# LonglongaaaGo/VSPBFR

Measured on AMD Instinct MI355X. Metric: restored 512x512 faces/sec, higher is better.
Workload: dtype f32; 1 GPU; restoration_test.py hot path A+B+C+D, batch 8/GPU, 512x512, 50-step DDPM CodeDiffuser + StyleGAN2 prior + RestoreNet forward, fp32, random-init weights; batch_per_gpu=8, with_style_sample=True, sampler=ddpm, overlap=A+B of batch i+1 on a second HIP stream under C+D of batch i, launch=eager (one host launch per kernel)

## Files before the change

### include/vspbfr_hip.h

```cpp
#ifndef VSPBFR_HIP_H
#define VSPBFR_HIP_H

#include <stdint.h>

#ifdef __cplusplus
extern "C" {
#endif

#define VSP_ABI_VERSION 4

#define VSP_OK 0
#define VSP_EINVAL (-1)
#define VSP_ELAUNCH (-2)
#define VSP_ENOTSUP (-3)

typedef void* vsp_stream_t;

int vsp_abi_version(void);
const char* vsp_last_error(void);
int vsp_device_count(void);
int vsp_struct_size(int which);

int vsp_fused_bias_act_f32(float* out, const float* x, const float* bias, const float* ref, int64_t n,
                           int step_b, int size_b, int act, int grad, float alpha, float scale,
                           vsp_stream_t stream);

typedef struct vsp_fir_epilogue {
  const float* plane_scale;
  const float* noise;
  const float* noise_w;
  const float* act_bias;
  const void* res1;
  const void* res2;
  int channels;
  int act;
  float slope;
  float gain;
  int flags;
} vsp_fir_epilogue;
#define VSP_FIR_SEPARABLE 1

int vsp_upfirdn2d_f32(float* out, const float* x, const float* kernel, int major, int in_h, int in_w,
                      int minor, int kh, int kw, int up_x, int up_y, int down_x, int down_y, int pad_x0,
                      int pad_x1, int pad_y0, int pad_y1, const vsp_fir_epilogue* epi ,
                      vsp_stream_t stream);

typedef struct vsp_conv_params {
  const float* x;
  const float* w;
  float* y;
  int B, Cin, H, W;
  int G, cout_g;
  int OH, OW;
  int KH, KW;
  int stride_y, stride_x;
  int dil[4];
  int pad_y[4];
  int pad_x[4];
  int y_ch, y_coff, y_h, y_w;
  int osy, osx, ooy, oox;
  const float* in_scale;
  int in_scale_bstride;
  const float* in_shift;
  const float* out_scale;
  const float* ch_scale;
  const float* ch_bias;
  int act1;
  const float* bias1;
  float slope1, gain1;
  const float* noise;
  const float* noise_w;
  int act2;
  const float* bias2;
  const float* prelu;
  float slope2, gain2;
  const float* res1;
  const float* res2;
  int res_ch, res_coff;
  int tile_hint;
  int x_ch, x_group_stride;
  int transposed;
  int io_bf16;
  int dil_by_input_quarter;
  int64_t w_bstride;
} vsp_conv_params;

int vsp_conv2d_f32(const vsp_conv_params* p, vsp_stream_t stream);
int vsp_conv2d_winograd_f32(const vsp_conv_params* p, vsp_stream_t stream);
int vsp_conv2d_winograd_chunk(void);
int vsp_conv2d_winograd_mbw(int cout_g);
int vsp_conv2d_winograd4_f32(const vsp_conv_params* p, float* work, size_t work_floats, vsp_stream_t stream);
size_t vsp_winograd4f_weight_floats(int cin, int cout);
int vsp_winograd4f_weight_f32(float* U, const float* wp, int cin, int cout, vsp_stream_t stream);
int vsp_conv2d_winograd4f_f32(const vsp_conv_params* params, vsp_stream_t stream);

size_t vsp_conv2d_winograd4_work_floats(const vsp_conv_params* p);
size_t vsp_winograd4_weight_floats(int cin, int cout);
int vsp_winograd4_weight_f32(float* U, const float* wp, int cin, int cout, vsp_stream_t stream);
int vsp_conv1x1_small_f32(float* y, const float* w, const float* x, const float* bias, int B, int Cout, int Cin, int P, int act,
                          float slope, float gain, vsp_stream_t stream);
int vsp_pack_weight_f32(float* wp, const float* w, int G, int cout_g, int cin, int KH, int KW, int adjoint, int flip, float scale,
                        vsp_stream_t stream);
size_t vsp_winograd_weight_floats(int G, int cin, int cout_g);
int vsp_winograd_weight_f32(float* U, const float* wp, int G, int cin, int cout_g, vsp_stream_t stream);
int vsp_conv2d_num_configs(void);
const char* vsp_conv2d_config_name(int i);

int vsp_conv2d_bf16(const vsp_conv_params* p, vsp_stream_t stream);

int vsp_conv2d_bf16x3(const vsp_conv_params* p, vsp_stream_t stream);

int vsp_conv2d_bf16rv(const vsp_conv_params* p, vsp_stream_t stream);
int vsp_conv2d_bf16dg(const vsp_conv_params* p, vsp_stream_t stream);

typedef struct vsp_gemm_params {
  const float* A;
  const float* Bm;
  float* C;
  int Z, M, N, K;
  int64_t a_zs, a_ms, a_ks;
  int64_t b_zs, b_ns, b_ks;
  int64_t c_zs, c_ms;
  float alpha;
  const float* bias;
  float bias_scale;
  int act;
  float slope, gain;
  int64_t bias_zs;
} vsp_gemm_params;

int vsp_gemm_f32(const vsp_gemm_params* p, vsp_stream_t stream);

int vsp_pixelnorm_dim1_f32(float* out, const float* x, int Z, int R, int C, float eps, vsp_stream_t stream);
int vsp_layernorm_f32(float* out, const float* x, const float* add, const float* gamma, const float* beta,
                      int rows, int cols, float eps, int post, float slope, float gain, vsp_stream_t stream);
int vsp_softmax_lastdim_f32(float* out, const float* x, int rows, int cols, vsp_stream_t stream);
int vsp_softmax_dim1_f32(float* out, const float* x, int Z, int R, int C, vsp_stream_t stream);
int vsp_film_f32(float* out, const float* h, const float* gamma, const float* beta, int64_t n,
                 vsp_stream_t stream);
int vsp_axpby_idx_f32(float* out, const float* x, const float* y, const float* a, const float* b, int idx,
                      int64_t n, vsp_stream_t stream);
int vsp_demod_f32(float* out, const float* style, const float* wsq, int B, int Cin, int Cout, float wscale,
                  float eps, vsp_stream_t stream);
typedef struct {
  const float* w;
  const float* bias;
  const float* wsq;
  float* mod;
  float* demod;
  int64_t src_off;
  int cin, cout;
  float alpha, bias_scale, wscale2;
  int pad_;
} vsp_style_layer;
int vsp_style_plan_f32(const vsp_style_layer* table, int L, const float* src, int B, int64_t bstride, int K, int max_cin, int max_cout,
                       float eps, vsp_stream_t stream);
int vsp_demod_weight_f32(float* out, float* wsq, const float* style, const float* w, int B, int Cin, int Cout, int K, float wscale,
                         float eps, vsp_stream_t stream);
int vsp_demod_weight_bwd_f32(float* dstyle, float* dw, const float* g, const float* out, const float* style, const float* wsq,
                             const float* w, int B, int Cin, int Cout, int K, float wscale, vsp_stream_t stream);
int vsp_demod_weight_bwd_acc_f32(float* dstyle, float* dw, const float* g, int g_stride, const float* out, const float* style,
                                 const float* wsq, const float* w, int B, int Cin, int Cout, int K, float wscale, int accumulate,
                                 vsp_stream_t stream);
int vsp_avgpool2x2_f32(float* out, const float* x, int64_t planes, int OH, int OW, vsp_stream_t stream);
int vsp_upsample_add_f32(float* out, const float* x, const float* y, int64_t planes, int IH, int IW, int OH,
                         int OW, vsp_stream_t stream);
int vsp_plane_mean_f32(float* out, const float* x, int64_t planes, int hw, vsp_stream_t stream);
int vsp_scale_add_f32(float* out, const float* x, const float* gate, const float* y, int64_t planes, int hw,
                      vsp_stream_t stream);
int vsp_subsample_f32(float* out, const float* x, int64_t planes, int IH, int IW, int s, vsp_stream_t stream);
int vsp_quantize_u8_nhwc(uint8_t* out, const float* x, int B, int C, int H, int W, float lo, float hi,
                         vsp_stream_t stream);
#define VSP_WIN_UNIFORM7 7
#define VSP_WIN_GAUSS11 11
size_t vsp_pair_stats_work_bytes(int B, int H, int W, int C, int window);
int vsp_pair_stats_u8(unsigned long long* sse, double* ssim, const uint8_t* a, const uint8_t* b, int B, int H, int W, int C,
                      int window, void* work, vsp_stream_t stream);
int vsp_resize_bilinear_f32(float* out, const float* x, int64_t planes, int IH, int IW, int OH, int OW, vsp_stream_t stream);
int vsp_e4e_codes_f32(float* out, const float* heads, const float* latent_avg, int B, int T, int D, vsp_stream_t stream);
int vsp_rows_concat_f32(float* out, int B, int T, int nseg, const float* const* src, const int* batch_stride, const int* token_stride,
                        const int* width, const int* flip, vsp_stream_t stream);
int vsp_add3_f32(float* out, const float* a, const float* b, const float* c, int64_t n, vsp_stream_t stream);

int vsp_pointwise_f32(float* y, const float* x, const float* w, const float* in_scale, const float* ch_bias,
                      const float* bias1, int act1, const float* bias2, int act2, const float* res, const float* up_src,
                      const float* up_kernel, int W, int B, int Cin, int Cout, int64_t HW, vsp_stream_t stream);

int vsp_tacc_scores_f32(float* score, const float* P, int ldp, int k_off, const float* eQ, const float* wq,
                        int wq_stride, float tfrac, int B, int n_tok, int dim, vsp_stream_t stream);
int vsp_tacc_chan_attn_f32(float* t, const float* P, int ldp, int q2_off, int v2_off, const float* ek,
                           const float* wk, int wk_stride, float tfrac, int B, int n_tok, int dim,
                           vsp_stream_t stream);
int vsp_tacc_tail_f32(float* y, float* pn, const float* P, int ldp, int k_off, int v_off, const float* eQ,
                      const float* wq , float tfrac, const float* t, const float* gamma,
                      const float* beta, const float* xold, const float* c1, const float* c2, int idx, int B, int n_tok,
                      int dim, vsp_stream_t stream);
int vsp_tacc_head_pre_f32(float* out, const float* e, const float* wcol, int w_stride, const float* ln_w,
                          const float* ln_b, int S, int M, int dim, float t_div, vsp_stream_t stream);

typedef struct vsp_tacc_block {
  const float* wcat;
  const float* eQ;
  const float* ek;
  const float* wq;
  const float* wk;
  const float* gamma;
  const float* beta;
  const float* wcat_frag;
} vsp_tacc_block;

typedef struct vsp_tacc_chain_params {
  int B, n_tok, dim, n_blocks;
  const vsp_tacc_block* blocks;
  float* x;
  float* work;
  size_t work_floats;
  int n_steps;
  const int* step;
  const int* coef_idx;
  const float* c1;
  const float* c2;
  float t_div;
  int head_steps;
} vsp_tacc_chain_params;

size_t vsp_tacc_chain_work_floats(int B);
int vsp_tacc_chain_f32(const vsp_tacc_chain_params* p, vsp_stream_t stream);

int vsp_convert_f32_to_bf16(uint16_t* out, const float* x, int64_t n, vsp_stream_t stream);
int vsp_convert_bf16_to_f32(float* out, const uint16_t* x, int64_t n, vsp_stream_t stream);
int vsp_upfirdn2d_bf16(uint16_t* out, const uint16_t* x, const float* kernel, int major, int in_h, int in_w, int minor,
                       int kh, int kw, int up_x, int up_y, int down_x, int down_y, int pad_x0, int pad_x1, int pad_y0,
                       int pad_y1, const vsp_fir_epilogue* epilogue, vsp_stream_t stream);
size_t vsp_modulate_weight_bf16_bytes(int G, int cin, int cout_g);
int vsp_modulate_weight_bf16(uint16_t* out, const float* wp, const float* style, int B, int64_t style_bstride, int G, int cin, int cout_g,
                             vsp_stream_t stream);
int vsp_pointwise_bf16(void* y, const void* x, const float* w, const float* in_scale, const float* ch_bias,
                       const float* bias1, int act1, const float* bias2, int act2, const float* res, const float* up_src,
                       const float* up_kernel, int W, int B, int Cin, int Cout, int64_t HW, vsp_stream_t stream);

typedef struct vsp_conv_wgrad_params {
  const float* x;
  const float* dy;
  float* dw;
  const float* x_scale;
  const float* dy_scale;
  int B, Cin_g, H, W, G, Cout_g, OH, OW, KH, KW, stride, dil, pad;
  int x_ch, x_coff;
  int dy_ch, dy_coff;
  int x_shared;
  int per_group_geometry;
  int dil_g[4], pad_g[4];
  int accumulate;
  float* work;
  size_t work_floats;
  float dw_scale;
} vsp_conv_wgrad_params;
size_t vsp_conv2d_wgrad_work_floats(const vsp_conv_wgrad_params* p);
int vsp_conv2d_wgrad_f32(const vsp_conv_wgrad_params* p, vsp_stream_t stream);
int vsp_plane_dot_f32(float* out, const float* a, const float* b, int64_t planes, int64_t n, vsp_stream_t stream);
int vsp_plane_dot_scale_f32(float* out, float* a, const float* b, const float* scale, int64_t planes, int64_t n, vsp_stream_t stream);
int vsp_noise_bias_act_f32(float* y, const float* x, const float* noise, const float* noise_w, const float* bias, int B, int C,
                           int64_t hw, float slope, float gain, vsp_stream_t stream);
int vsp_noise_dot_f32(float* out, const float* gx, const float* noise, int B, int C, int64_t hw, vsp_stream_t stream);
int vsp_smart_tail_bwd_f32(float* g1, float* db1, float* db2, float* dnw, const float* g, const float* y, const float* noise,
                           const float* noise_w, const float* bias2, int B, int C, int64_t hw, float slope, float gain,
                           vsp_stream_t stream);
int vsp_channel_sum_f32(float* out, const float* x, int B, int C, int64_t hw, vsp_stream_t stream);

int vsp_affine_sample_f32(float* out, const float* x, const float* theta, int B, int C, int IH, int IW, int OH, int OW,
                          vsp_stream_t stream);
int vsp_affine_sample_bwd_f32(float* gx, const float* gout, const float* theta, int B, int C, int IH, int IW, int OH, int OW,
                              vsp_stream_t stream);
int vsp_color_affine_f32(float* y, const float* x, const float* M, const float* t, int B, int64_t HW, vsp_stream_t stream);

int vsp_maxpool2d_f32(float* out, const float* x, int64_t planes, int H, int W, int OH, int OW, int k, int s, int p,
                      vsp_stream_t stream);
int vsp_maxpool2d_bwd_f32(float* dx, const float* dy, const float* x, int64_t planes, int H, int W, int OH, int OW, int k, int s,
                          int p, vsp_stream_t stream);
int vsp_lpips_layer_f32(float* out, const float* f0, const float* f1, const float* w, int B, int C, int HW, vsp_stream_t stream);
int vsp_lpips_layer_bwd_f32(float* df1, const float* f0, const float* f1, const float* w, const float* gout, int B, int C, int HW,
                            vsp_stream_t stream);
int vsp_resize_bilinear_bwd_f32(float* dx, const float* dy, int64_t planes, int IH, int IW, int OH, int OW, vsp_stream_t stream);

#define VSP_NOISE_MAX_SEGMENTS 64
int vsp_keyed_fill_f32(float* out, int B, const int64_t* seg_elems, const int32_t* seg_ids, int n_seg, uint64_t seed,
                       int64_t image_index0, const int64_t* image_index0_dev, int dist, vsp_stream_t stream);

#define VSP_DEGRADE_MAX_KSIZE 41
#define VSP_DEGRADE_MAX_SIZE 2048
#define VSP_DEGRADE_MAX_ITEMS 1024
#define VSP_DEGRADE_HAZE 1
#define VSP_DEGRADE_GREY 2
#define VSP_DEGRADE_NOISE_KEY 0x44475244u

typedef struct vsp_degrade_item {
  int64_t tap_off;
  int64_t pix_off;
  int64_t jpg_off;
  int64_t sample;
  int32_t src;
  int32_t ksize;
  int32_t dh, dw;
  int32_t quality;
  int32_t flags;
  int32_t mcu0;
  int32_t slot;
  float alpha;
  float sigma;
} vsp_degrade_item;

int vsp_degrade_gt_f32(float* out, const uint8_t* hwc, const float* in, const int32_t* grey, int B, int H, int W, vsp_stream_t stream);
int vsp_degrade_blur_f32(float* out, const float* gt, const float* taps, const vsp_degrade_item* items, int n, int B, int H, int W,
                         vsp_stream_t stream);
int vsp_degrade_down_u8(uint8_t* lq, float* pre, const float* blurred, const float* noise, const vsp_degrade_item* items, int n, int H,
                        int W, int max_pixels, uint64_t seed, int64_t step, vsp_stream_t stream);
int vsp_degrade_jpeg_u8(uint8_t* lq, uint8_t* work, const vsp_degrade_item* items, int n, int total_mcus, int max_pixels,
                        vsp_stream_t stream);
int vsp_degrade_up_f32(float* out, const uint8_t* lq, const vsp_degrade_item* items, int n, int H, int W, vsp_stream_t stream);

#define VSP_RESAMPLE_PRECISION_BITS 22
#define VSP_RESAMPLE_MAX_TAPS 97
#define VSP_RESAMPLE_MAX_SIDE 8192
#define VSP_RESAMPLE_MAX_ITEMS 65535
#define VSP_RESAMPLE_FLIP 1
#define VSP_RESAMPLE_COPY 2

typedef struct vsp_resample_item {
  int64_t src_off;
  int64_t work_off;
  int64_t hco, vco;
  int32_t sw, sh;
  int32_t nw, nh;
  int32_t x0, y0;
  int32_t row0, row1;
  int32_t hk, vk;
  int32_t flags;
  int32_t pad_;
} vsp_resample_item;

size_t vsp_lanczos_work_bytes(int rows, int W);
int vsp_lanczos_resize_u8(uint8_t* out_u8, float* out_f32, const uint8_t* src, size_t src_bytes, const int32_t* coef, size_t coef_ints,
                          uint8_t* work, size_t work_bytes, const vsp_resample_item* items, const vsp_resample_item* items_dev, int n,
                          int H, int W, vsp_stream_t stream);

typedef struct vsp_resample_dst {
  int64_t out_off;
  int32_t W, H;
} vsp_resample_dst;

int vsp_lanczos_resize_ragged_u8(uint8_t* out, size_t out_bytes, const uint8_t* src, size_t src_bytes, const int32_t* coef, size_t coef_ints,
                                 uint8_t* work, size_t work_bytes, const vsp_resample_item* items, const vsp_resample_item* items_dev,
                                 const vsp_resample_dst* dst, const vsp_resample_dst* dst_dev, int n, vsp_stream_t stream);

#define VSP_PNG_SEG_ROWS 8
#define VSP_PNG_MAX_ROW_BYTES 3072
#define VSP_PNG_MAX_H 32768
#define VSP_PNG_MAX_BATCH 65535
size_t vsp_png_segment_bound(int rows, int W, int C);
size_t vsp_png_bound(int H, int W, int C);
int vsp_png_encode_u8(uint8_t* out, size_t out_capacity, int32_t* seg_bytes, uint32_t* seg_adler, const uint8_t* src, int B, int H, int W,
                      int C, vsp_stream_t stream);

#define VSP_PNG_RAGGED_SEG_BYTES 24576
#define VSP_PNG_RAGGED_SLOT_BYTES 24588
#define VSP_PNG_RAGGED_MAX_ROW_BYTES (1 << 20)
#define VSP_PNG_RAGGED_MAX_IMAGES 4096
#define VSP_PNG_RAGGED_MAX_SEGMENTS 65535

typedef struct vsp_png_item {
  int64_t src_off;
  int64_t out_off;
  int32_t h, w;
  int32_t seg0;
  int32_t row0;
} vsp_png_item;

int vsp_png_ragged_segments(int H, int W, int C);
size_t vsp_png_ragged_image_bound(int H, int W, int C);
size_t vsp_png_ragged_work_bytes(int64_t segments, int64_t rows);
int vsp_png_encode_ragged_u8(uint8_t* out, size_t out_bytes, int32_t* idat_bytes, uint32_t* seg_adler, uint8_t* work, size_t work_bytes,
                             const uint8_t* src, size_t src_bytes, const vsp_png_item* items, const vsp_png_item* items_dev, int n, int C,
                             vsp_stream_t stream);

#define VSP_NIQE_BLOCK 96
#define VSP_NIQE_FEATURES 36
#define VSP_NIQE_GAMMAS 9801
size_t vsp_niqe_work_bytes(int B, int H, int W, int crop_border);
int vsp_niqe_features_u8(double* features, double* moments_or_null, float* sharpness, const uint8_t* img, int B, int H, int W,
                         int crop_border, const double* rgam_table, void* work, vsp_stream_t stream);

#define VSP_FACE_TILE 32
#define VSP_FACE_MAX_SIDE 8192
#define VSP_FACE_MAX_ITEMS 65535
#define VSP_FACE_MAX_RAMP 65536

typedef struct vsp_face_item {
  int64_t src_off;
  int64_t tab_off;
  int32_t h, w;
  int32_t x0, y0;
  int32_t nx, ny;
} vsp_face_item;

typedef struct vsp_face_tile {
  int64_t dst_off;
  int32_t h, w;
  int32_t x0, y0;
  int32_t face0;
  int32_t nfaces;
} vsp_face_tile;

int vsp_face_crop_u8(uint8_t* out_u8, float* out_f32, const uint8_t* src, size_t src_bytes, const int32_t* tables, const int32_t* tables_dev,
                     size_t table_ints, const vsp_face_item* items, const vsp_face_item* items_dev, int n, int S, int border_r, int border_g,
                     int border_b, vsp_stream_t stream);
int vsp_face_paste_u8(uint8_t* photos, size_t photo_bytes, const uint8_t* crops, size_t crop_bytes, const int32_t* tables,
                      const int32_t* tables_dev, size_t table_ints, const vsp_face_item* items, const vsp_face_item* items_dev, int n, int S,
                      const vsp_face_tile* tiles, const vsp_face_tile* tiles_dev, int ntiles, const int32_t* tile_faces,
                      const int32_t* tile_faces_dev, size_t tile_face_ints, const uint16_t* ramp, const uint16_t* ramp_dev, int ramp_len,
                      vsp_stream_t stream);

#define VSP_FACE_AA_MAX_REACH 23
#define VSP_FACE_AA_MAX_RANGE (1 << 18)

typedef struct vsp_face_aa_item {
  int64_t src_off;
  int64_t tab_off;
  int64_t fwd_off;
  int32_t h, w;
  int32_t x0, y0;
  int32_t nx, ny;
  int32_t sx0, sy0;
  int32_t snx, sny;
  int32_t reach;
  int32_t pad_;
} vsp_face_aa_item;

int vsp_face_crop_aa_u8(uint8_t* out_u8, float* out_f32, const uint8_t* src, size_t src_bytes, const int32_t* tables, const int32_t* tables_dev,
                        size_t table_ints, const int32_t* fwd, const int32_t* fwd_dev, size_t fwd_ints, const vsp_face_aa_item* items,
                        const vsp_face_aa_item* items_dev, int n, int S, int border_r, int border_g, int border_b, vsp_stream_t stream);
int vsp_face_paste_aa_u8(uint8_t* photos, size_t photo_bytes, const uint8_t* crops, size_t crop_bytes, const int32_t* tables,
                         const int32_t* tables_dev, size_t table_ints, const int32_t* fwd, const int32_t* fwd_dev, size_t fwd_ints,
                         const vsp_face_aa_item* items, const vsp_face_aa_item* items_dev, int n, int S, const vsp_face_tile* tiles,
                         const vsp_face_tile* tiles_dev, int ntiles, const int32_t* tile_faces, const int32_t* tile_faces_dev,
                         size_t tile_face_ints, const uint16_t* ramp, const uint16_t* ramp_dev, int ramp_len, vsp_stream_t stream);

#define VSP_COLOR_FIX_STATS 0
#define VSP_COLOR_FIX_WAVELET 1
#define VSP_COLOR_FIX_MAX_LEVELS 6
#define VSP_COLOR_FIX_STATS_MAX_SIDE 1024

int vsp_color_fix_u8(const uint8_t* crop, const uint8_t* restored, uint8_t* out, int F, int S, int mode, int levels,
                     const vsp_face_item* items, const vsp_face_item* items_dev, const int32_t* tables, const int32_t* tables_dev,
                     size_t table_ints, void* scratch, size_t scratch_bytes, vsp_stream_t stream);

#define VSP_JPEG_444 0
#define VSP_JPEG_420 2
#define VSP_JPEG_MAX_ITEMS 65535
#define VSP_JPEG_BLOCK_BOUND 416

typedef struct vsp_jpeg_item {
  int64_t src_off;
  int64_t out_off;
  int32_t h, w;
  int32_t interval0;
  int32_t pad_;
} vsp_jpeg_item;

int vsp_jpeg_intervals(int h, int w, int restart, int subsampling);
size_t vsp_jpeg_interval_bound(int mcus, int subsampling);
size_t vsp_jpeg_image_bound(int h, int w, int restart, int subsampling);
int vsp_jpeg_encode_u8(uint8_t* out, size_t out_bytes, int32_t* totals, uint8_t* work, size_t work_bytes, int32_t* interval_ws,
                       const uint8_t* src, size_t src_bytes, const vsp_jpeg_item* items, const vsp_jpeg_item* items_dev, int n,
                       int quality, int subsampling, int restart, vsp_stream_t stream);

#define VSP_JPEG_DEC_TABLE_BYTES 1824
#define VSP_JPEG_DEC_MAX_SCAN_BYTES 0x0FFFFFFF
#define VSP_JPEG_DEC_COEF_LIMIT 16383
#define VSP_JPEG_DEC_NO_EOI 1
#define VSP_JPEG_DEC_STRAY_MARKER 2
#define VSP_JPEG_DEC_RST_ORDER 4
#define VSP_JPEG_DEC_RST_COUNT 8
#define VSP_JPEG_DEC_BAD_CODE 16
#define VSP_JPEG_DEC_BAD_CATEGORY 32
#define VSP_JPEG_DEC_RUN 64
#define VSP_JPEG_DEC_BLOCK_COUNT 128
#define VSP_JPEG_DEC_COEF_RANGE 256

typedef struct vsp_jpeg_dec_item {
  int64_t in_off;
  int64_t out_off;
  int64_t work_off;
  int32_t in_len;
  int32_t h, w;
  int32_t subsampling;
  int32_t restart;
  int32_t interval0;
} vsp_jpeg_dec_item;

size_t vsp_jpeg_decode_work_bytes(int h, int w, int in_len, int subsampling, int restart, int sub_bytes);
int vsp_jpeg_decode_u8(uint8_t* out, size_t out_bytes, int32_t* status, int32_t* rounds, uint8_t* work, size_t work_bytes, const uint8_t* in,
                       size_t in_bytes, const vsp_jpeg_dec_item* items, const vsp_jpeg_dec_item* items_dev, const uint8_t* tables,
                       const uint8_t* tables_dev, int n, int sub_bytes, vsp_stream_t stream);

#ifdef __cplusplus
}
#endif
#endif
```

### vspbfr_amd/_lib.py

```python
import ctypes as C
import os

import torch

from .photo import FaceAAItem, FaceItem, FaceTile
from .resample import ResampleDst, ResampleItem

_HERE = os.path.dirname(os.path.abspath(__file__))
LIB_PATH = os.environ.get("VSPBFR_HIP_LIB", os.path.join(_HERE, "lib", "libvspbfr_hip.so"))



def tune_env(name, default=None):
    if os.environ.get("VSP_TUNE", "0") in ("", "0"):
        return default
    return os.environ.get(name, default)


ABI_VERSION = 4
c_float_p = C.c_void_p


class FirEpilogue(C.Structure):
    _fields_ = [
        ("plane_scale", C.c_void_p), ("noise", C.c_void_p), ("noise_w", C.c_void_p), ("act_bias", C.c_void_p),
        ("res1", C.c_void_p), ("res2", C.c_void_p),
        ("channels", C.c_int), ("act", C.c_int), ("slope", C.c_float), ("gain", C.c_float), ("flags", C.c_int),
    ]


FIR_SEPARABLE = 1


class ConvParams(C.Structure):
    _fields_ = [
        ("x", C.c_void_p), ("w", C.c_void_p), ("y", C.c_void_p),
        ("B", C.c_int), ("Cin", C.c_int), ("H", C.c_int), ("W", C.c_int),
        ("G", C.c_int), ("cout_g", C.c_int),
        ("OH", C.c_int), ("OW", C.c_int),
        ("KH", C.c_int), ("KW", C.c_int),
        ("stride_y", C.c_int), ("stride_x", C.c_int),
        ("dil", C.c_int * 4), ("pad_y", C.c_int * 4), ("pad_x", C.c_int * 4),
        ("y_ch", C.c_int), ("y_coff", C.c_int), ("y_h", C.c_int), ("y_w", C.c_int),
        ("osy", C.c_int), ("osx", C.c_int), ("ooy", C.c_int), ("oox", C.c_int),
        ("in_scale", C.c_void_p), ("in_scale_bstride", C.c_int), ("in_shift", C.c_void_p),
        ("out_scale", C.c_void_p), ("ch_scale", C.c_void_p), ("ch_bias", C.c_void_p),
        ("act1", C.c_int), ("bias1", C.c_void_p), ("slope1", C.c_float), ("gain1", C.c_float),
        ("noise", C.c_void_p), ("noise_w", C.c_void_p),
        ("act2", C.c_int), ("bias2", C.c_void_p), ("prelu", C.c_void_p), ("slope2", C.c_float), ("gain2", C.c_float),
        ("res1", C.c_void_p), ("res2", C.c_void_p), ("res_ch", C.c_int), ("res_coff", C.c_int),
        ("tile_hint", C.c_int), ("x_ch", C.c_int), ("x_group_stride", C.c_int), ("transposed", C.c_int),
        ("io_bf16", C.c_int),
        ("dil_by_input_quarter", C.c_int),
        ("w_bstride", C.c_int64),
    ]


class ConvWgradParams(C.Structure):
    _fields_ = [("x", C.c_void_p), ("dy", C.c_void_p), ("dw", C.c_void_p), ("x_scale", C.c_void_p), ("dy_scale", C.c_void_p)] + [
        (n, C.c_int) for n in ("B", "Cin_g", "H", "W", "G", "Cout_g", "OH", "OW", "KH", "KW", "stride", "dil", "pad", "x_ch", "x_coff", "dy_ch",
                               "dy_coff", "x_shared", "per_group_geometry")] + [("dil_g", C.c_int * 4), ("pad_g", C.c_int * 4),
                                                                                ("accumulate", C.c_int), ("work", C.c_void_p),
                                                                                ("work_floats", C.c_size_t), ("dw_scale", C.c_float)]


class TaccBlock(C.Structure):
    _fields_ = [(n, C.c_void_p) for n in ("wcat", "eQ", "ek", "wq", "wk", "gamma", "beta", "wcat_frag")]


class TaccChainParams(C.Structure):
    _fields_ = [
        ("B", C.c_int), ("n_tok", C.c_int), ("dim", C.c_int), ("n_blocks", C.c_int),
        ("blocks", C.POINTER(TaccBlock)), ("x", C.c_void_p), ("work", C.c_void_p), ("work_floats", C.c_size_t),
        ("n_steps", C.c_int), ("step", C.POINTER(C.c_int)), ("coef_idx", C.POINTER(C.c_int)),
        ("c1", C.c_void_p), ("c2", C.c_void_p), ("t_div", C.c_float), ("head_steps", C.c_int),
    ]


class GemmParams(C.Structure):
    _fields_ = [
        ("A", C.c_void_p), ("Bm", C.c_void_p), ("C", C.c_void_p),
        ("Z", C.c_int), ("M", C.c_int), ("N", C.c_int), ("K", C.c_int),
        ("a_zs", C.c_int64), ("a_ms", C.c_int64), ("a_ks", C.c_int64),
        ("b_zs", C.c_int64), ("b_ns", C.c_int64), ("b_ks", C.c_int64),
        ("c_zs", C.c_int64), ("c_ms", C.c_int64),
        ("alpha", C.c_float), ("bias", C.c_void_p), ("bias_scale", C.c_float),
        ("act", C.c_int), ("slope", C.c_float), ("gain", C.c_float), ("bias_zs", C.c_int64),
    ]


class DegradeItem(C.Structure):
    _fields_ = [("tap_off", C.c_int64), ("pix_off", C.c_int64), ("jpg_off", C.c_int64), ("sample", C.c_int64)] + [
        (n, C.c_int32) for n in ("src", "ksize", "dh", "dw", "quality", "flags", "mcu0", "slot")] + [("alpha", C.c_float), ("sigma", C.c_float)]


class JpegItem(C.Structure):
    _fields_ = [("src_off", C.c_int64), ("out_off", C.c_int64), ("h", C.c_int32), ("w", C.c_int32), ("interval0", C.c_int32), ("pad_", C.c_int32)]


class PngItem(C.Structure):
    _fields_ = [("src_off", C.c_int64), ("out_off", C.c_int64), ("h", C.c_int32), ("w", C.c_int32), ("seg0", C.c_int32), ("row0", C.c_int32)]


class JpegDecItem(C.Structure):
    _fields_ = [("in_off", C.c_int64), ("out_off", C.c_int64), ("work_off", C.c_int64)] + [
        (n, C.c_int32) for n in ("in_len", "h", "w", "subsampling", "restart", "interval0")]


DEGRADE_HAZE, DEGRADE_GREY = 1, 2
DEGRADE_MAX_KSIZE, DEGRADE_MAX_SIZE, DEGRADE_MAX_ITEMS = 41, 2048, 1024
WIN_UNIFORM7, WIN_GAUSS11 = 7, 11

_i, _i64, _f, _p = C.c_int, C.c_int64, C.c_float, C.c_void_p

SIGNATURES = {
    "vsp_abi_version": [],
    "vsp_device_count": [],
    "vsp_struct_size": [_i],
    "vsp_fused_bias_act_f32": [_p, _p, _p, _p, _i64, _i, _i, _i, _i, _f, _f, _p],
    "vsp_upfirdn2d_f32": [_p, _p, _p] + [_i] * 14 + [C.POINTER(FirEpilogue), _p],
    "vsp_conv2d_f32": [C.POINTER(ConvParams), _p],
    "vsp_conv2d_num_configs": [],
    "vsp_gemm_f32": [C.POINTER(GemmParams), _p],
    "vsp_pixelnorm_dim1_f32": [_p, _p, _i, _i, _i, _f, _p],
    "vsp_layernorm_f32": [_p, _p, _p, _p, _p, _i, _i, _f, _i, _f, _f, _p],
    "vsp_softmax_lastdim_f32": [_p, _p, _i, _i, _p],
    "vsp_softmax_dim1_f32": [_p, _p, _i, _i, _i, _p],
    "vsp_film_f32": [_p, _p, _p, _p, _i64, _p],
    "vsp_axpby_idx_f32": [_p, _p, _p, _p, _p, _i, _i64, _p],
    "vsp_demod_f32": [_p, _p, _p, _i, _i, _i, _f, _f, _p],
    "vsp_style_plan_f32": [_p, _i, _p, _i, _i64, _i, _i, _i, _f, _p],
    "vsp_demod_weight_f32": [_p, _p, _p, _p, _i, _i, _i, _i, _f, _f, _p],
    "vsp_demod_weight_bwd_f32": [_p, _p, _p, _p, _p, _p, _p, _i, _i, _i, _i, _f, _p],
    "vsp_demod_weight_bwd_acc_f32": [_p, _p, _p, _i, _p, _p, _p, _p, _i, _i, _i, _i, _f, _i, _p],
    "vsp_avgpool2x2_f32": [_p, _p, _i64, _i, _i, _p],
    "vsp_upsample_add_f32": [_p, _p, _p, _i64, _i, _i, _i, _i, _p],
    "vsp_e4e_codes_f32": [_p, _p, _p, _i, _i, _i, _p],
    "vsp_rows_concat_f32": [_p, _i, _i, _i, C.POINTER(C.c_void_p), C.POINTER(_i), C.POINTER(_i), C.POINTER(_i), C.POINTER(_i), _p],
    "vsp_resize_bilinear_f32": [_p, _p, _i64, _i, _i, _i, _i, _p],
    "vsp_plane_mean_f32": [_p, _p, _i64, _i, _p],
    "vsp_scale_add_f32": [_p, _p, _p, _p, _i64, _i, _p],
    "vsp_subsample_f32": [_p, _p, _i64, _i, _i, _i, _p],
    "vsp_add3_f32": [_p, _p, _p, _p, _i64, _p],
    "vsp_pointwise_f32": [_p, _p, _p, _p, _p, _p, _i, _p, _i, _p, _p, _p, _i, _i, _i, _i, _i64, _p],
    "vsp_quantize_u8_nhwc": [_p, _p, _i, _i, _i, _i, _f, _f, _p],
    "vsp_tacc_scores_f32": [_p, _p, _i, _i, _p, _p, _i, _f, _i, _i, _i, _p],
    "vsp_tacc_chan_attn_f32": [_p, _p, _i, _i, _i, _p, _p, _i, _f, _i, _i, _i, _p],
    "vsp_tacc_tail_f32": [_p, _p, _p, _i, _i, _i, _p, _p, _f, _p, _p, _p, _p, _p, _p, _i, _i, _i, _i, _p],
    "vsp_tacc_head_pre_f32": [_p, _p, _p, _i, _p, _p, _i, _i, _i, _f, _p],
    "vsp_tacc_chain_f32": [_p, _p],
    "vsp_conv2d_winograd_f32": [_p, _p],
    "vsp_conv2d_bf16": [_p, _p],
    "vsp_conv2d_bf16x3": [_p, _p],
    "vsp_conv2d_bf16rv": [_p, _p],
    "vsp_conv2d_bf16dg": [_p, _p],
    "vsp_affine_sample_f32": [_p, _p, _p, _i, _i, _i, _i, _i, _i, _p],
    "vsp_affine_sample_bwd_f32": [_p, _p, _p, _i, _i, _i, _i, _i, _i, _p],
    "vsp_color_affine_f32": [_p, _p, _p, _p, _i, _i64, _p],
    "vsp_maxpool2d_f32": [_p, _p, _i64, _i, _i, _i, _i, _i, _i, _i, _p],
    "vsp_maxpool2d_bwd_f32": [_p, _p, _p, _i64, _i, _i, _i, _i, _i, _i, _i, _p],
    "vsp_lpips_layer_f32": [_p, _p, _p, _p, _i, _i, _i, _p],
    "vsp_lpips_layer_bwd_f32": [_p, _p, _p, _p, _p, _i, _i, _i, _p],
    "vsp_resize_bilinear_bwd_f32": [_p, _p, _i64, _i, _i, _i, _i, _p],
    "vsp_conv2d_wgrad_f32": [C.POINTER(ConvWgradParams), _p],
    "vsp_plane_dot_f32": [_p, _p, _p, _i64, _i64, _p],
    "vsp_channel_sum_f32": [_p, _p, _i, _i, _i64, _p],
    "vsp_noise_bias_act_f32": [_p, _p, _p, _p, _p, _i, _i, _i64, C.c_float, C.c_float, _p],
    "vsp_noise_dot_f32": [_p, _p, _p, _i, _i, _i64, _p],
    "vsp_smart_tail_bwd_f32": [_p, _p, _p, _p, _p, _p, _p, _p, _p, _i, _i, _i64, C.c_float, C.c_float, _p],
    "vsp_plane_dot_scale_f32": [_p, _p, _p, _p, _i64, _i64, _p],
    "vsp_convert_f32_to_bf16": [_p, _p, _i64, _p],
    "vsp_convert_bf16_to_f32": [_p, _p, _i64, _p],
    "vsp_upfirdn2d_bf16": [_p, _p, _p] + [_i] * 14 + [C.POINTER(FirEpilogue), _p],
    "vsp_pointwise_bf16": [_p, _p, _p, _p, _p, _p, _i, _p, _i, _p, _p, _p, _i, _i, _i, _i, _i64, _p],
    "vsp_keyed_fill_f32": [_p, _i, C.POINTER(C.c_int64), C.POINTER(C.c_int32), _i, C.c_uint64, _i64, _p, _i, _p],
    "vsp_conv1x1_small_f32": [_p, _p, _p, _p, _i, _i, _i, _i, _i, _f, _f, _p],
    "vsp_pack_weight_f32": [_p, _p, _i, _i, _i, _i, _i, _i, _i, _f, _p],
    "vsp_winograd_weight_f32": [_p, _p, _i, _i, _i, _p],
    "vsp_winograd4_weight_f32": [_p, _p, _i, _i, _p],
    "vsp_conv2d_winograd4_f32": [_p, _p, C.c_size_t, _p],
    "vsp_winograd4f_weight_f32": [_p, _p, _i, _i, _p],
    "vsp_conv2d_winograd4f_f32": [_p, _p],
    "vsp_modulate_weight_bf16": [_p, _p, _p, _i, _i64, _i, _i, _i, _p],
    "vsp_conv2d_winograd_chunk": [],
    "vsp_conv2d_winograd_mbw": [_i],
    "vsp_degrade_gt_f32": [_p, _p, _p, _p, _i, _i, _i, _p],
    "vsp_degrade_blur_f32": [_p, _p, _p, _p, _i, _i, _i, _i, _p],
    "vsp_degrade_down_u8": [_p, _p, _p, _p, _p, _i, _i, _i, _i, C.c_uint64, _i64, _p],
    "vsp_degrade_jpeg_u8": [_p, _p, _p, _i, _i, _i, _p],
    "vsp_degrade_up_f32": [_p, _p, _p, _i, _i, _i, _p],
    "vsp_pair_stats_u8": [_p, _p, _p, _p, _i, _i, _i, _i, _i, _p, _p],
    "vsp_lanczos_resize_u8": [_p, _p, _p, C.c_size_t, _p, C.c_size_t, _p, C.c_size_t, _p, _p, _i, _i, _i, _p],
    "vsp_lanczos_resize_ragged_u8": [_p, C.c_size_t, _p, C.c_size_t, _p, C.c_size_t, _p, C.c_size_t, _p, _p, _p, _p, _i, _p],
    "vsp_png_encode_u8": [_p, C.c_size_t, _p, _p, _p, _i, _i, _i, _i, _p],
    "vsp_png_ragged_segments": [_i, _i, _i],
    "vsp_png_encode_ragged_u8": [_p, C.c_size_t, _p, _p, _p, C.c_size_t, _p, C.c_size_t, _p, _p, _i, _i, _p],
    "vsp_niqe_features_u8": [_p, _p, _p, _p, _i, _i, _i, _i, _p, _p, _p],
    "vsp_face_crop_u8": [_p, _p, _p, C.c_size_t, _p, _p, C.c_size_t, _p, _p, _i, _i, _i, _i, _i, _p],
    "vsp_face_paste_u8": [_p, C.c_size_t, _p, C.c_size_t, _p, _p, C.c_size_t, _p, _p, _i, _i, _p, _p, _i, _p, _p, C.c_size_t, _p, _p, _i, _p],
    "vsp_face_crop_aa_u8": [_p, _p, _p, C.c_size_t, _p, _p, C.c_size_t, _p, _p, C.c_size_t, _p, _p, _i, _i, _i, _i, _i, _p],
    "vsp_face_paste_aa_u8": [_p, C.c_size_t, _p, C.c_size_t, _p, _p, C.c_size_t, _p, _p, C.c_size_t, _p, _p, _i, _i, _p, _p, _i, _p, _p,
                             C.c_size_t, _p, _p, _i, _p],
    "vsp_color_fix_u8": [_p, _p, _p, _i, _i, _i, _i, _p, _p, _p, _p, C.c_size_t, _p, C.c_size_t, _p],
    "vsp_jpeg_intervals": [_i, _i, _i, _i],
    "vsp_jpeg_encode_u8": [_p, C.c_size_t, _p, _p, C.c_size_t, _p, _p, C.c_size_t, _p, _p, _i, _i, _i, _i, _p],
    "vsp_jpeg_decode_u8": [_p, C.c_size_t, _p, _p, _p, C.c_size_t, _p, C.c_size_t, _p, _p, _p, _p, _i, _i, _p],
}
_CHARP = {"vsp_last_error": [], "vsp_conv2d_config_name": [_i]}
_SIZET = {"vsp_tacc_chain_work_floats": [_i], "vsp_conv2d_wgrad_work_floats": [C.POINTER(ConvWgradParams)],
          "vsp_winograd_weight_floats": [_i, _i, _i], "vsp_winograd4_weight_floats": [_i, _i], "vsp_winograd4f_weight_floats": [_i, _i],
          "vsp_conv2d_winograd4_work_floats": [_p], "vsp_modulate_weight_bf16_bytes": [_i, _i, _i],
          "vsp_pair_stats_work_bytes": [_i, _i, _i, _i, _i], "vsp_lanczos_work_bytes": [_i, _i],
          "vsp_png_segment_bound": [_i, _i, _i], "vsp_png_bound": [_i, _i, _i],
          "vsp_png_ragged_image_bound": [_i, _i, _i], "vsp_png_ragged_work_bytes": [_i64, _i64],
          "vsp_niqe_work_bytes": [_i, _i, _i, _i],
          "vsp_jpeg_interval_bound": [_i, _i], "vsp_jpeg_image_bound": [_i, _i, _i, _i],
          "vsp_jpeg_decode_work_bytes": [_i, _i, _i, _i, _i, _i]}


def _load():
    if not os.path.exists(LIB_PATH):
        raise ImportError(
            f"vspbfr_amd: HIP library not found at {LIB_PATH}. Build it with `python -c 'import __graft_entry__ as g; "
            f"g.build()'` or `make -C vspbfr_amd/csrc`; there is no CPU fallback.")
    lib = C.CDLL(LIB_PATH)
    for name, args in SIGNATURES.items():
        fn = getattr(lib, name)
        fn.argtypes = args
        fn.restype = C.c_int
    for name, args in _CHARP.items():
        fn = getattr(lib, name)
        fn.argtypes = args
        fn.restype = C.c_char_p
    for name, args in _SIZET.items():
        fn = getattr(lib, name)
        fn.argtypes = args
        fn.restype = C.c_size_t
    if lib.vsp_abi_version() != ABI_VERSION:
        raise ImportError(f"vspbfr_amd: ABI version {lib.vsp_abi_version()} != {ABI_VERSION}")
    for which, st in ((0, FirEpilogue), (1, ConvParams), (2, GemmParams), (3, TaccBlock), (4, TaccChainParams),
                      (5, ConvWgradParams), (6, DegradeItem), (7, ResampleItem), (8, FaceItem), (9, FaceTile), (10, FaceAAItem), (11, JpegItem), (12, JpegDecItem),
                      (13, ResampleDst), (14, PngItem)):
        if lib.vsp_struct_size(which) != C.sizeof(st):
            raise ImportError(f"vspbfr_amd: struct layout mismatch for {st.__name__}: "
                              f"C {lib.vsp_struct_size(which)} vs ctypes {C.sizeof(st)}")
    return lib


lib = _load()


def last_error():
    return lib.vsp_last_error().decode("utf-8", "replace")


def check(rc, what):
    if rc != 0:
        raise RuntimeError(f"{what} failed (code {rc}): {last_error()}")


def exported_symbols():
    return sorted(list(SIGNATURES) + list(_CHARP) + list(_SIZET))
```

### vspbfr_amd/csrc/conv_igemm.hip

```cpp
#include "conv_kernel.h"
#include <cstdlib>
#include <cstring>

namespace vspconv {
extern const Cfg kCfgsA[];
extern const int kNumA;
extern const Cfg kCfgsB[];
extern const int kNumB;
extern const Cfg kCfgsC[];
extern const int kNumC;
extern const Cfg kCfgsD[];
extern const int kNumD;
extern const Cfg kCfgsE[];
extern const int kNumE;
extern const Cfg kCfgsF[];
extern const int kNumF;
extern const Cfg kCfgsG[];
extern const int kNumG;
extern const Cfg kCfgsP[];
extern const int kNumP;
}

namespace {

using vspconv::Cfg;
using vspconv::ConvK;

__device__ float kConst[8] = {1.f, 0.f, 1.f, 0.f, 0.f, 0.f, 0.f, 0.f};

constexpr int kMaxCfgs = 192;
static Cfg kCfgs[kMaxCfgs];
static int kNumCfgs = 0;

static void build_table() {
  if (kNumCfgs) return;
  using namespace vspconv;
  const struct { const Cfg* cfgs; int count; } units[] = {{kCfgsA, kNumA}, {kCfgsB, kNumB}, {kCfgsC, kNumC}, {kCfgsD, kNumD},
                                                          {kCfgsE, kNumE}, {kCfgsF, kNumF}, {kCfgsG, kNumG}, {kCfgsP, kNumP}};
  int n = 0;
  for (const auto& u : units)
    for (int i = 0; i < u.count && n < kMaxCfgs; ++i) kCfgs[n++] = u.cfgs[i];
  kNumCfgs = n;
}

constexpr size_t kMaxLds = 100 * 1024;
constexpr size_t kMaxLdsPipe = 160 * 1024;

struct Plan {
  int cfg;
  int tw_log2, th, tiles_x, tiles_y, co_tiles;
  bool dg;
  int strip_col, strip_row;
  size_t lds;
  int ps;
};

static int ilog2_ceil(int v) {
  int l = 0;
  while ((1 << l) < v) ++l;
  return l;
}

static int host_round_pitch(int n, int odd) {
  if (odd) return n | 1;
  int p = (n & ~31) + 16;
  return p >= n ? p : p + 32;
}

struct CfgKind {
  bool tc, dg, kg, fg;
};
static CfgKind cfg_kind(const Cfg& k) {
  const size_t n = strlen(k.name);
  const char last = k.name[n - 1];
  return {last == 't', last == 'd', last == 'a', n >= 2 && k.name[n - 2] == 'f'};
}

static bool make_plan(const vsp_conv_params& p, int c, Plan* out) {
  const Cfg& k = kCfgs[c];
  const CfgKind kind = cfg_kind(k);
  const bool tc = kind.tc;
  if (tc != (p.transposed != 0)) return false;
  const bool kg = kind.kg;
  if (kg != (p.dil_by_input_quarter != 0)) return false;
  const bool dg = kind.dg || kg;
  if (dg) {
    if (p.G != 4 || p.x_group_stride != 0 || p.stride_y != 1 || p.stride_x != 1 || p.KH != 3 || p.KW != 3) return false;
    for (int g = 0; g < 4; ++g)
      if (p.pad_y[g] != p.dil[g] || p.pad_x[g] != p.dil[g]) return false;
  }
  const int CO_T = 16 * k.MB * k.WM, NPIX = tc ? 16 * k.WN * (k.NB / 4) : 16 * k.NB * k.WN;
  const int WS = (CO_T % 32 == 0) ? CO_T + 16 : CO_T;
  int twl = ilog2_ceil(p.OW);
  int cap = NPIX >= 256 ? 5 : 4;
  if (k.PF == 3 && dg) cap = NPIX >= 512 ? 5 : 4;
  if (twl > cap) twl = cap;
  if ((1 << twl) > NPIX) twl = ilog2_ceil(NPIX);
  const bool fg = k.PF == 3 && kind.fg;
  if (fg) {
    twl = 4;
    if (!dg || p.dil[0] != 1 || p.dil[1] != 2 || p.dil[2] != 4 || p.dil[3] != 8) return false;
  }
  const int TW = 1 << twl, TH = NPIX / TW;
  int dmax = 1;
  for (int g = 0; g < (p.G > 4 ? 1 : p.G); ++g) dmax = p.dil[g] > dmax ? p.dil[g] : dmax;
  const int PH = tc ? TH + 1 : (TH - 1) * p.stride_y + (p.KH - 1) * dmax + 1;
  const int PW = tc ? TW + 1 : (TW - 1) * p.stride_x + (p.KW - 1) * dmax + 1;
  if (PW > 256 || PH * PW >= 65536) return false;
  int plane = PH * PW;
  out->strip_col = -1;
  out->strip_row = 0;
  out->tiles_x = (p.OW + TW - 1) / TW;
  out->tiles_y = (p.OH + TH - 1) / TH;
  if (tc && (NPIX <= 128 || k.PF == 3) && p.H % TH == 0 && p.W % TW == 0) {
    out->tiles_x = p.W / TW;
    out->tiles_y = p.H / TH;
    out->strip_col = (p.H + NPIX - 1) / NPIX;
    out->strip_row = (p.W + 1 + NPIX - 1) / NPIX;
    if ((NPIX + 1) * 2 > plane) plane = (NPIX + 1) * 2;
  }
  if (k.PF == 3) {
    if (p.KH != 3 || p.KW != 3 || p.cout_g % 4 != 0 || !vsp::aligned16(p.w) || p.in_shift || p.Cin % k.CK != 0) return false;
    if (kg && (p.Cin % 16 != 0 || (p.Cin / 4) % k.CK != 0)) return false;
    const int NW = k.WM * k.WN, wpc = k.CK >= NW ? 1 : NW / k.CK;
    const int nrow = (plane + 63) / 64;
    const int ps = host_round_pitch(k.PMAX * wpc * 64, !tc && p.stride_x != 1);
    if (nrow > k.PMAX * wpc) return false;
    const size_t lds = 2 * ((size_t)9 * k.CK * WS + (size_t)k.CK * ps) * sizeof(float);
    if (lds > kMaxLdsPipe) return false;
    out->cfg = c; out->tw_log2 = twl; out->th = TH;
    out->co_tiles = dg ? (p.cout_g + 15) / 16 : (p.cout_g + CO_T - 1) / CO_T;
    out->dg = dg; out->lds = lds; out->ps = ps;
    return true;
  }
  const int PS = host_round_pitch(plane, !tc && p.stride_x != 1);
  if (k.PF == 2 && (p.in_shift || p.cout_g % 4 != 0 || !vsp::aligned16(p.w) || p.KH * p.KW > 9)) return false;
  size_t lds = ((size_t)p.KH * p.KW * k.CK * WS + (size_t)(k.PF == 2 ? 2 : 1) * k.CK * PS) * sizeof(float);
  const size_t red = (size_t)(k.WK - 1) * k.WM * k.WN * k.MB * k.NB * 4 * 64 * sizeof(float);
  if (red > lds) lds = red;
  if (lds > kMaxLds) return false;
  out->cfg = c;
  out->tw_log2 = twl;
  out->th = TH;
  out->co_tiles = dg ? (p.cout_g + 15) / 16 : (p.cout_g + CO_T - 1) / CO_T;
  out->dg = dg;
  out->lds = lds;
  return true;
}

static double plan_cost(const vsp_conv_params& p, const Plan& pl) {
  const Cfg& k = kCfgs[pl.cfg];
  const int waves = k.WM * k.WN * k.WK;
  const double blocks = ((double)pl.tiles_x * pl.tiles_y + (pl.strip_col > 0 ? pl.strip_col + pl.strip_row : 0)) * pl.co_tiles * (pl.dg ? 1 : p.G) * p.B;
  const int cin_pad = (p.Cin + k.CK - 1) / k.CK * k.CK;
  const double ksteps = (double)p.KH * p.KW * cin_pad / 4.0;
  const double mfma_cyc = ksteps * k.MB * k.NB * 32.0 / k.WK;
  const double reads = ksteps * (k.MB + k.NB) * 8.0 / k.WK;
  const double chunks = (double)cin_pad / k.CK;
  const double stage = chunks * 2500.0;
  int per_cu = (int)(160 * 1024 / (pl.lds + 1024));
  if (per_cu > 4) per_cu = 4;
  if (per_cu < 1) per_cu = 1;
  const double wps = per_cu * waves / 4.0;
  double t_block = mfma_cyc * (wps < 1.0 ? 1.0 : wps) + (wps >= 2.0 ? 0.15 : 1.0) * stage + 0.05 * reads;
  const double slots = 256.0 * per_cu;
  const double rounds = blocks / slots;
  const double full = (rounds < 1.0) ? 1.0 : rounds;
  if (rounds < 1.0) {
    const double occ = blocks / 256.0;
    const double w = occ * waves / 4.0;
    t_block = mfma_cyc * (w < 1.0 ? 1.0 : w) + stage + 0.05 * reads;
  }
  return full * t_block;
}

static const float* device_consts() {
  static const float* cache[64] = {};
  int dev = 0;
  if (hipGetDevice(&dev) != hipSuccess || dev < 0 || dev >= 64) {
    vsp::set_error("hipGetDevice failed");
    return nullptr;
  }
  if (!cache[dev]) {
    void* ptr = nullptr;
    hipError_t e = hipGetSymbolAddress(&ptr, HIP_SYMBOL(kConst));
    if (e != hipSuccess) {
      vsp::set_error("hipGetSymbolAddress(kConst): %s", hipGetErrorString(e));
      return nullptr;
    }
    const float init[8] = {1.f, 0.f, 1.f, 0.f, 0.2f, 0.01f, 0.f, 0.f};
    e = hipMemcpy(ptr, init, sizeof(init), hipMemcpyHostToDevice);
    if (e != hipSuccess) {
      vsp::set_error("hipMemcpy(kConst): %s", hipGetErrorString(e));
      return nullptr;
    }
    cache[dev] = static_cast<const float*>(ptr);
  }
  return cache[dev];
}

static const float* slope_slot(const float* kc, float slope) {
  if (slope == 0.2f) return kc + 4;
  if (slope == 0.01f) return kc + 5;
  if (slope == 1.f) return kc;
  if (slope == 0.f) return kc + 1;
  return nullptr;
}

}

static int validate_conv(const vsp_conv_params& p, int* x_ch_out, bool* empty, bool allow_w_bstride = false) {
  *empty = false;
  VSP_REQUIRE(p.x && p.w && p.y, "conv2d: null tensor pointer");
  VSP_REQUIRE(p.B >= 0 && p.Cin >= 1 && p.H >= 1 && p.W >= 1, "conv2d: bad input dims B=%d Cin=%d H=%d W=%d", p.B,
              p.Cin, p.H, p.W);
  VSP_REQUIRE(p.G >= 1 && p.G <= 1024 && p.cout_g >= 1, "conv2d: bad group spec G=%d cout_g=%d", p.G, p.cout_g);
  VSP_REQUIRE(p.x_group_stride >= 0 && p.x_ch >= 0, "conv2d: negative x_ch / x_group_stride");
  VSP_REQUIRE(p.w_bstride == 0 || allow_w_bstride, "conv2d: per-image weights (w_bstride) are served by vsp_conv2d_bf16 with io_bf16 = 1 only");
  const int x_ch = p.x_ch > 0 ? p.x_ch : p.Cin;
  VSP_REQUIRE((int64_t)(p.G - 1) * p.x_group_stride + p.Cin <= x_ch, "conv2d: group input channels exceed x_ch=%d", x_ch);
  VSP_REQUIRE(p.x_group_stride == 0 || !p.in_shift, "conv2d: an input shift is not supported with grouped input");
  VSP_REQUIRE(p.KH >= 1 && p.KW >= 1 && p.KH * p.KW <= 49, "conv2d: unsupported kernel %dx%d", p.KH, p.KW);
  VSP_REQUIRE(p.stride_y >= 1 && p.stride_x >= 1 && p.stride_x <= 2 && p.stride_y <= 2, "conv2d: stride must be 1 or 2");
  VSP_REQUIRE(p.dil_by_input_quarter == 0 || (p.dil_by_input_quarter == 1 && p.G == 4 && p.x_group_stride == 0 && p.Cin % 16 == 0 && !p.transposed),
              "conv2d: dil_by_input_quarter needs G = 4 blocks of output channels over one shared input with Cin %% 16 == 0");
  VSP_REQUIRE(p.OH >= 0 && p.OW >= 0, "conv2d: negative output size");
  VSP_REQUIRE(p.osy >= 1 && p.osx >= 1 && p.ooy >= 0 && p.oox >= 0, "conv2d: bad output stride/offset");
  VSP_REQUIRE(!p.noise || p.noise_w, "conv2d: noise given without noise_w");
  VSP_REQUIRE(p.act2 != 2 || p.prelu, "conv2d: act2=prelu without slopes");
  for (int g = 0; g < (p.G > 4 ? 1 : p.G); ++g) VSP_REQUIRE(p.dil[g] >= 1, "conv2d: dilation must be >= 1");
  if (p.B == 0 || p.OH == 0 || p.OW == 0) {
    *empty = true;
    return VSP_OK;
  }
  const int Cout = p.G * p.cout_g;
  VSP_REQUIRE(p.y_coff >= 0 && p.y_coff + Cout <= p.y_ch, "conv2d: output channel window [%d,%d) outside %d", p.y_coff,
              p.y_coff + Cout, p.y_ch);
  VSP_REQUIRE((p.OH - 1) * p.osy + p.ooy < p.y_h && (p.OW - 1) * p.osx + p.oox < p.y_w,
              "conv2d: output positions exceed the %dx%d output tensor", p.y_h, p.y_w);
  VSP_REQUIRE((int64_t)p.y_ch * p.y_h * p.y_w < ((int64_t)1 << 31) && (int64_t)x_ch * p.H * p.W < ((int64_t)1 << 31),
              "conv2d: one image must hold fewer than 2^31 elements");
  if (p.res1 || p.res2)
    VSP_REQUIRE(p.res_coff >= 0 && p.res_coff + Cout <= p.res_ch, "conv2d: residual channel window out of range");

  *x_ch_out = x_ch;
  return VSP_OK;
}

static int fill_convk(const vsp_conv_params& p, int x_ch, ConvK& q) {
  q.x = p.x; q.w = p.w; q.y = p.y;
  q.B = p.B; q.Cin = p.Cin; q.H = p.H; q.W = p.W; q.G = p.G; q.cout_g = p.cout_g;
  q.OH = p.OH; q.OW = p.OW; q.KH = p.KH; q.KW = p.KW; q.sy = p.stride_y; q.sx = p.stride_x;
  for (int g = 0; g < 4; ++g) { q.dil[g] = p.dil[g]; q.pady[g] = p.pad_y[g]; q.padx[g] = p.pad_x[g]; }
  q.y_ch = p.y_ch; q.y_coff = p.y_coff; q.y_h = p.y_h; q.y_w = p.y_w;
  q.osy = p.osy; q.osx = p.osx; q.ooy = p.ooy; q.oox = p.oox;
  q.in_scale = p.in_scale; q.in_scale_bstride = p.in_scale_bstride; q.in_shift = p.in_shift;
  const float* kc = device_consts();
  VSP_REQUIRE(kc != nullptr, "conv2d: cannot resolve device constants: %s", vsp_last_error());
  const float* kOne = kc;
  const float* kZero = kc + 1;
  auto sel = [](const float* ptr, const float* dflt, const float** outp, int* outs) {
    *outp = ptr ? ptr : dflt;
    *outs = ptr ? 1 : 0;
  };
  sel(p.out_scale, kOne, &q.osp, &q.oss);
  sel(p.ch_scale, kOne, &q.csp, &q.css);
  sel(p.ch_bias, kZero, &q.cbp, &q.cbs);
  sel(p.act1 ? p.bias1 : nullptr, kZero, &q.b1p, &q.b1s);
  q.s1 = p.act1 ? p.slope1 : 1.f;
  q.g1 = p.act1 ? p.gain1 : 1.f;
  sel(p.noise, kZero, &q.nzp, &q.nzs);
  q.nwp = p.noise ? p.noise_w : kZero;
  sel(p.act2 == 1 ? p.bias2 : nullptr, kZero, &q.b2p, &q.b2s);
  if (p.act2 == 2) {
    q.s2p = p.prelu; q.s2s = 1; q.g2 = 1.f;
  } else if (p.act2 == 1) {
    const float* slot = slope_slot(kc, p.slope2);
    VSP_REQUIRE(slot != nullptr, "conv2d: unsupported act2 slope %g (supported: 0.2, 0.01, 0, 1)", p.slope2);
    q.s2p = slot; q.s2s = 0; q.g2 = p.gain2;
  } else {
    q.s2p = kOne; q.s2s = 0; q.g2 = 1.f;
  }
  sel(p.res1, kZero, &q.r1p, &q.r1s);
  sel(p.res2, kZero, &q.r2p, &q.r2s);
  q.res_ch = p.res_ch; q.res_coff = p.res_coff;
  q.x_ch = x_ch;
  q.x_gs = p.x_group_stride;
  return VSP_OK;
}

static int conv_front(const vsp_conv_params& p, ConvK& q, bool* empty, bool allow_w_bstride = false) {
  int x_ch = 0;
  if (int rc = validate_conv(p, &x_ch, empty, allow_w_bstride)) return rc;
  if (*empty) return VSP_OK;
  if (int rc = fill_convk(p, x_ch, q)) return rc;
  static const int dbg = vsp::tune_env("VSP_CONV_DBG") ? atoi(vsp::tune_env("VSP_CONV_DBG")) : 0;
  q.dbg = dbg;
  const float* kc = device_consts();
  const bool affine = p.in_shift != nullptr, style = p.in_scale && !affine, scaled = p.in_scale && affine;
  q.wtp = style ? p.in_scale : kc;       q.wt_cs = style ? 1 : 0;    q.wt_bs = style ? p.in_scale_bstride : 0;
  q.wcp = scaled ? p.in_scale : kc;      q.wc_cs = scaled ? 1 : 0;   q.wc_bs = scaled ? p.in_scale_bstride : 0;
  q.wshp = affine ? p.in_shift : kc + 1; q.wsh_cs = affine ? 1 : 0;
  q.bf_isc_s = p.in_scale ? 1 : 0;
  q.bf_ish_s = affine ? 1 : 0;
  return VSP_OK;
}

static int require_dilation_groups(const char* who, const vsp_conv_params& p, int n, int dmax, bool pow2) {
  for (int g = 0; g < n; ++g)
    VSP_REQUIRE(p.dil[g] >= 1 && p.dil[g] <= dmax && (!pow2 || (p.dil[g] & (p.dil[g] - 1)) == 0) && p.pad_y[g] == p.dil[g] && p.pad_x[g] == p.dil[g],
                "%s: group %d needs a dilation of %s and padding = dilation (got dilation %d, padding %d/%d)", who, g,
                pow2 ? "1, 2, 4 or 8" : "1 to 64", p.dil[g], p.pad_y[g], p.pad_x[g]);
  return VSP_OK;
}

static int require_dense_output(const char* who, const vsp_conv_params& p, bool same_size) {
  const bool dense = p.osy == 1 && p.osx == 1 && p.ooy == 0 && p.oox == 0;
  if (!same_size) {
    VSP_REQUIRE(dense, "%s: dense output only", who);
    return VSP_OK;
  }
  VSP_REQUIRE(dense && p.OH == p.H && p.OW == p.W, "%s: dense same-size output only: the output size must equal the input size", who);
  return VSP_OK;
}

static int require_input_under_2gib(const char* who, const vsp_conv_params& p) {
  VSP_REQUIRE((double)(p.x_ch > 0 ? p.x_ch : p.Cin) * p.H * p.W * 4 < 2147483648.0,
              "%s: one input image must be smaller than 2 GiB (32-bit buffer offsets)", who);
  return VSP_OK;
}

static int normalise_transposed(const char* who, vsp_conv_params& p, bool exact) {
  VSP_REQUIRE(p.KH == 3 && p.KW == 3 && p.G == 1, "%s: transposed mode needs a 3x3 kernel and G = 1", who);
  VSP_REQUIRE(!p.noise && !p.res1 && !p.res2, "%s: transposed mode has no noise / residual epilogue", who);
  const int oh = 2 * p.H + 1, ow = 2 * p.W + 1;
  VSP_REQUIRE(exact ? (p.y_h == oh && p.y_w == ow) : (p.y_h >= oh && p.y_w >= ow), "%s: transposed output must %s (2H+1)x(2W+1)", who,
              exact ? "be" : "hold");
  p.stride_y = p.stride_x = 1;
  p.dil[0] = 1;
  p.pad_y[0] = p.pad_x[0] = 1;
  p.OH = p.H + 1;
  p.OW = p.W + 1;
  p.osy = p.osx = 2;
  p.ooy = p.oox = 0;
  return VSP_OK;
}

extern "C" int vsp_conv2d_num_configs(void) {
  build_table();
  return kNumCfgs + 1;
}
extern "C" const char* vsp_conv2d_config_name(int i) {
  build_table();
  return (i >= 0 && i < kNumCfgs) ? kCfgs[i].name : (i == kNumCfgs ? "smallmap" : "");
}

extern "C" int vsp_conv2d_winograd_chunk(void) { return vspconv::wino_chunk(); }
extern "C" int vsp_conv2d_winograd_mbw(int cout_g) { return vspconv::wino_mbw(cout_g); }

extern "C" int vsp_conv2d_winograd_f32(const vsp_conv_params* pp, vsp_stream_t stream) {
  const char* who = "conv2d_winograd";
  VSP_REQUIRE(pp != nullptr, "conv2d_winograd: null params");
  const vsp_conv_params& p = *pp;
  VSP_REQUIRE(!p.transposed && p.G >= 1 && p.G <= 4 && p.KH == 3 && p.KW == 3 && p.stride_y == 1 && p.stride_x == 1 &&
                  p.x_group_stride == 0,
              "conv2d_winograd: only 3x3, stride 1, at most four groups over one shared input");
  if (int rc = require_dilation_groups(who, p, p.G, 8, true)) return rc;
  VSP_REQUIRE(p.io_bf16 == 0, "conv2d_winograd: fp32 activations only (io_bf16 is served by vsp_conv2d_bf16)");
  VSP_REQUIRE(p.dil_by_input_quarter == 0, "conv2d_winograd: dil_by_input_quarter is served by vsp_conv2d_f32");
  if (int rc = require_dense_output(who, p, true)) return rc;
  VSP_REQUIRE(vsp::aligned16(p.w), "conv2d_winograd: transformed weights must be 16-byte aligned");
  VSP_REQUIRE((int64_t)16 * p.Cin * p.cout_g < ((int64_t)1 << 31), "conv2d_winograd: weight tensor too large");
  if (int rc = require_input_under_2gib(who, p)) return rc;
  VSP_REQUIRE(p.tile_hint >= 0 && p.tile_hint <= 3, "conv2d_winograd: tile_hint names the kernel form: 0 automatic, 1 task list, 2 row owner, 3 register-resident U");
  ConvK q{};
  bool empty = false;
  if (int rc = conv_front(p, q, &empty)) return rc;
  if (empty) return VSP_OK;
  if (int rc = vspconv::wino_launch(q, p.tile_hint, vsp::as_stream(stream))) return rc;
  return vsp::check_launch(who);
}

extern "C" size_t vsp_winograd4_weight_floats(int cin, int cout) { return vspconv::wino4_weight_floats(cin, cout); }

extern "C" int vsp_winograd4_weight_f32(float* U, const float* wp, int cin, int cout, vsp_stream_t stream) {
  VSP_REQUIRE(U && wp && cin >= 1 && cout >= 1, "winograd4_weight: bad arguments");
  if (int rc = vspconv::wino4_weight_launch(U, wp, cin, cout, vsp::as_stream(stream))) return rc;
  return vsp::check_launch("winograd4_weight");
}

extern "C" size_t vsp_conv2d_winograd4_work_floats(const vsp_conv_params* pp) {
  return pp ? vspconv::wino4_work_floats(pp->B, pp->Cin, pp->H, pp->W) : 0;
}

extern "C" int vsp_conv2d_winograd4_f32(const vsp_conv_params* pp, float* work, size_t work_floats, vsp_stream_t stream) {
  const char* who = "conv2d_winograd4";
  VSP_REQUIRE(pp != nullptr && work != nullptr, "conv2d_winograd4: null params / work buffer");
  const vsp_conv_params& p = *pp;
  VSP_REQUIRE(!p.transposed && p.G == 1 && p.KH == 3 && p.KW == 3 && p.stride_y == 1 && p.stride_x == 1 && p.dil[0] == 1 &&
                  p.pad_y[0] == 1 && p.pad_x[0] == 1,
              "conv2d_winograd4: one group, 3x3, stride 1, dilation 1, padding 1");
  VSP_REQUIRE(p.io_bf16 == 0 && p.dil_by_input_quarter == 0 && p.in_shift == nullptr, "conv2d_winograd4: fp32, no affine input shift");
  if (int rc = require_dense_output(who, p, true)) return rc;
  VSP_REQUIRE(vsp::aligned16(p.w) && vsp::aligned16(work), "conv2d_winograd4: weights and work buffer must be 16-byte aligned");
  VSP_REQUIRE(work_floats >= vspconv::wino4_work_floats(p.B, p.Cin, p.H, p.W), "conv2d_winograd4: work buffer too small");
  VSP_REQUIRE((int64_t)vspconv::wino4_work_floats(1, p.Cin, p.H, p.W) * 4 < ((int64_t)1 << 40), "conv2d_winograd4: image too large");
  ConvK q{};
  bool empty = false;
  if (int rc = conv_front(p, q, &empty)) return rc;
  if (empty) return VSP_OK;
  if (!vspconv::wino4_eligible(q))
    return vsp::fail(VSP_ENOTSUP, "conv2d_winograd4: needs Cin %% 4 == 0, H, W %% 4 == 0, dense 16-byte aligned output / noise / residual planes");
  if (int rc = vspconv::wino4_launch(q, work, p.in_scale, p.in_scale ? p.in_scale_bstride : 0, vsp::as_stream(stream))) return rc;
  return vsp::check_launch(who);
}

extern "C" size_t vsp_winograd4f_weight_floats(int cin, int cout) { return vspconv::wino4f_weight_floats(cin, cout); }

extern "C" int vsp_winograd4f_weight_f32(float* U, const float* wp, int cin, int cout, vsp_stream_t stream) {
  VSP_REQUIRE(U && wp && cin >= 1 && cout >= 1, "winograd4f_weight: bad arguments");
  if (int rc = vspconv::wino4f_weight_launch(U, wp, cin, cout, vsp::as_stream(stream))) return rc;
  return vsp::check_launch("winograd4f_weight");
}

extern "C" int vsp_conv2d_winograd4f_f32(const vsp_conv_params* pp, vsp_stream_t stream) {
  const char* who = "conv2d_winograd4f";
  VSP_REQUIRE(pp != nullptr, "conv2d_winograd4f: null params");
  const vsp_conv_params& p = *pp;
  VSP_REQUIRE(!p.transposed && p.G >= 1 && p.G <= 4 && p.KH == 3 && p.KW == 3 && p.stride_y == 1 && p.stride_x == 1,
              "conv2d_winograd4f: 3x3, stride 1, one group or up to four dilation groups over one shared input");
  if (int rc = require_dilation_groups(who, p, p.G, 8, true)) return rc;
  VSP_REQUIRE(p.io_bf16 == 0 && p.dil_by_input_quarter == 0 && p.in_shift == nullptr, "conv2d_winograd4f: fp32, no affine input shift");
  if (int rc = require_dense_output(who, p, true)) return rc;
  VSP_REQUIRE(vsp::aligned16(p.w), "conv2d_winograd4f: weights must be 16-byte aligned");
  ConvK q{};
  bool empty = false;
  if (int rc = conv_front(p, q, &empty)) return rc;
  if (empty) return VSP_OK;
  if (!vspconv::wino4f_eligible(q))
    return vsp::fail(VSP_ENOTSUP, "conv2d_winograd4f: needs Cin %% 8 == 0 (<= 512), H, W %% (4 x dilation) == 0, W >= 16, groups over one shared input, dense 16-byte aligned input / output / noise / residual planes < 2 GiB per image");
  if (int rc = vspconv::wino4f_launch(q, vsp::as_stream(stream))) return rc;
  return vsp::check_launch(who);
}

enum Bf16Kernel { kBf16General, kBf16Split, kBf16RowVector, kBf16DilationGroups };
static int conv2d_bf16_impl(const vsp_conv_params* pp, vsp_stream_t stream, Bf16Kernel kern);
extern "C" int vsp_conv2d_bf16(const vsp_conv_params* pp, vsp_stream_t stream) { return conv2d_bf16_impl(pp, stream, kBf16General); }
extern "C" int vsp_conv2d_bf16x3(const vsp_conv_params* pp, vsp_stream_t stream) { return conv2d_bf16_impl(pp, stream, kBf16Split); }
extern "C" int vsp_conv2d_bf16rv(const vsp_conv_params* pp, vsp_stream_t stream) { return conv2d_bf16_impl(pp, stream, kBf16RowVector); }
extern "C" int vsp_conv2d_bf16dg(const vsp_conv_params* pp, vsp_stream_t stream) { return conv2d_bf16_impl(pp, stream, kBf16DilationGroups); }

static int conv2d_bf16_impl(const vsp_conv_params* pp, vsp_stream_t stream, Bf16Kernel kern) {
  const char* who = "conv2d_bf16";
  VSP_REQUIRE(pp != nullptr, "conv2d_bf16: null params");
  vsp_conv_params pcopy = *pp;
  int mode = 0;
  VSP_REQUIRE(pcopy.KH == 3 && pcopy.KW == 3 && pcopy.G >= 1, "conv2d_bf16: 3x3 kernels only");
  if (pcopy.transposed) {
    mode = 2;
    if (int rc = normalise_transposed(who, pcopy, true)) return rc;
  } else if (pcopy.stride_y == 2 && pcopy.stride_x == 2) {
    mode = 1;
    VSP_REQUIRE(pcopy.dil[0] == 1 && pcopy.pad_y[0] == pcopy.pad_x[0] && (pcopy.pad_y[0] == 0 || pcopy.pad_y[0] == 1),
                "conv2d_bf16: stride 2 needs dilation 1 and padding 0 or 1");
    VSP_REQUIRE(pcopy.G == 1 || pcopy.x_group_stride > 0, "conv2d_bf16: stride-2 groups need their own input slices");
    VSP_REQUIRE(pcopy.OH <= (pcopy.H + 2 * pcopy.pad_y[0] - 3) / 2 + 1 && pcopy.OW <= (pcopy.W + 2 * pcopy.pad_x[0] - 3) / 2 + 1,
                "conv2d_bf16: output larger than the stride-2 convolution of the input");
  } else {
    VSP_REQUIRE(pcopy.stride_y == 1 && pcopy.stride_x == 1, "conv2d_bf16: stride must be 1 or 2");
    VSP_REQUIRE(pcopy.G <= 4 || pcopy.x_group_stride > 0, "conv2d_bf16: more than four groups need their own input slices");
    if (int rc = require_dilation_groups(who, pcopy, pcopy.G > 4 ? 1 : pcopy.G, 64, false)) return rc;
  }
  const vsp_conv_params& p = pcopy;
  if (mode != 2)
    if (int rc = require_dense_output(who, p, mode == 0)) return rc;
  VSP_REQUIRE(vsp::aligned16(p.w), "conv2d_bf16: packed weights must be 16-byte aligned");
  VSP_REQUIRE(p.Cin % 8 == 0, "conv2d_bf16: Cin must be a multiple of 8 (got %d)", p.Cin);
  if (int rc = require_input_under_2gib(who, p)) return rc;
  if (p.w_bstride != 0) {
    VSP_REQUIRE(kern == kBf16General && p.io_bf16 == 1, "conv2d_bf16: per-image weights need the general bf16 kernel with bf16 activations");
    VSP_REQUIRE(p.w_bstride > 0 && p.w_bstride % 16 == 0, "conv2d_bf16: w_bstride must be a positive multiple of 16 bytes");
    VSP_REQUIRE(!p.in_scale && !p.in_shift, "conv2d_bf16: per-image weights carry the style: in_scale / in_shift must be NULL");
    VSP_REQUIRE((p.W & 1) == 0 && (reinterpret_cast<uintptr_t>(p.x) & 3) == 0, "conv2d_bf16: per-image weights need even rows (pixel-pair staging)");
  }
  VSP_REQUIRE((int64_t)p.G * p.cout_g <= 65535 && p.B <= 65535, "conv2d_bf16: grid too large");
  VSP_REQUIRE(!(kern == kBf16Split && p.io_bf16), "conv2d_bf16x3: the split-precision form keeps fp32 activations (io_bf16 = 0)");
  VSP_REQUIRE(p.io_bf16 == 0 || p.io_bf16 == 1, "conv2d_bf16: io_bf16 must be 0 or 1");
  VSP_REQUIRE(p.dil_by_input_quarter == 0, "conv2d_bf16: dil_by_input_quarter is served by vsp_conv2d_f32");
  ConvK q{};
  bool empty = false;
  if (int rc = conv_front(p, q, &empty, true)) return rc;
  if (empty) return VSP_OK;
  q.in_scale = p.in_shift ? q.wcp : q.wtp;
  q.in_scale_bstride = p.in_shift ? q.wc_bs : q.wt_bs;
  q.in_shift = q.wshp;
  q.io_bf16 = p.io_bf16;
  q.w_bs = p.w_bstride / 16;
  const hipStream_t s = vsp::as_stream(stream);
  switch (kern) {
    case kBf16DilationGroups:
      if (mode != 0 || !vspconv::bf16dg_eligible(q)) return VSP_ENOTSUP;
      if (int rc = vspconv::bf16dg_launch(q, p.act1 != 0 || p.act2 != 0 || p.noise != nullptr, s)) return rc;
      return vsp::check_launch("conv2d_bf16dg");
    case kBf16RowVector:
      if (mode != 0 || !vspconv::bf16rv_eligible(q)) return VSP_ENOTSUP;
      if (int rc = vspconv::bf16rv_launch(q, p.tile_hint, s)) return rc;
      return vsp::check_launch("conv2d_bf16rv");
    case kBf16Split:
      if (int rc = vspconv::bf16_launch_split(q, mode, p.tile_hint, s)) return rc;
      return vsp::check_launch("conv2d_bf16x3");
    case kBf16General: break;
  }
  if (int rc = vspconv::bf16_launch(q, mode, p.tile_hint, s)) return rc;
  return vsp::check_launch(who);
}

extern "C" int vsp_conv2d_f32(const vsp_conv_params* pp, vsp_stream_t stream) {
  const char* who = "conv2d";
  VSP_REQUIRE(pp != nullptr, "conv2d: null params");
  VSP_REQUIRE(pp->io_bf16 == 0, "conv2d: fp32 activations only (io_bf16 is served by vsp_conv2d_bf16)");
  build_table();
  vsp_conv_params pcopy = *pp;
  if (pcopy.transposed)
    if (int rc = normalise_transposed(who, pcopy, false)) return rc;
  const vsp_conv_params& p = pcopy;
  if (int rc = require_input_under_2gib(who, p)) return rc;
  VSP_REQUIRE((double)p.KH * p.KW * p.Cin * p.cout_g * 4 < 2147483648.0, "conv2d: one group's weights must be smaller than 2 GiB (32-bit buffer offsets)");
  ConvK q{};
  bool empty = false;
  if (int rc = conv_front(p, q, &empty)) return rc;
  if (empty) return VSP_OK;
  {
    const int sm = kNumCfgs + 1;
    const bool named = p.tile_hint == sm, preferred = p.tile_hint == -sm;
    const bool guess = p.tile_hint == 0 && (int64_t)p.B * p.OH * p.OW <= 256 && (int64_t)p.Cin * p.KH * p.KW >= 1024;
    if ((named || preferred || guess) && !p.dil_by_input_quarter) {
      if (vspconv::smallmap_eligible(q, p.transposed != 0)) return vspconv::smallmap_launch(q, vsp::as_stream(stream));
      VSP_REQUIRE(!named, "conv2d: configuration smallmap does not fit this problem (Cin %% 16 == 0, at most 8192 output positions, not transposed)");
    }
  }
  Plan best{};
  bool found = false;
  if (p.tile_hint > 0) {
    VSP_REQUIRE(p.tile_hint <= kNumCfgs, "conv2d: tile_hint %d out of range", p.tile_hint);
    found = make_plan(p, p.tile_hint - 1, &best);
    VSP_REQUIRE(found, "conv2d: configuration %s does not fit this problem", kCfgs[p.tile_hint - 1].name);
  } else if (p.tile_hint < 0 && -p.tile_hint <= kNumCfgs) {
    found = make_plan(p, -p.tile_hint - 1, &best);
  }
  if (!found) {
    double best_cost = 0.0;
    for (int c = 0; c < kNumCfgs; ++c) {
      Plan pl{};
      const CfgKind kind = cfg_kind(kCfgs[c]);
      if (p.dil_by_input_quarter ? !kind.kg : (kind.dg || kCfgs[c].PF == 3)) continue;
      if (!make_plan(p, c, &pl)) continue;
      const double cost = p.dil_by_input_quarter ? (double)c : plan_cost(p, pl);
      if (!found || cost < best_cost) {
        best = pl;
        best_cost = cost;
        found = true;
      }
    }
    if (!found) return vsp::fail(VSP_ENOTSUP, "conv2d: no tile configuration fits (KH=%d dil=%d)", p.KH, p.dil[0]);
  }
  const Cfg& k = kCfgs[best.cfg];
  const int CO_T = 16 * k.MB * k.WM;
  const int64_t gy = best.dg ? best.co_tiles : (int64_t)best.co_tiles * p.G;
  VSP_REQUIRE(gy <= 65535 && p.B <= 65535, "conv2d: grid too large");

  q.tw_log2 = best.tw_log2; q.th = best.th; q.tiles_x = best.tiles_x; q.tiles_y = best.tiles_y;
  q.strip_col = best.strip_col;
  q.co_tiles = best.co_tiles;
  q.w_vec4 = (p.cout_g % 4 == 0) && (CO_T % 4 == 0) && vsp::aligned16(p.w) ? 1 : 0;
  q.ps_odd = !p.transposed && p.stride_x != 1;

  if (k.PF == 3) {
    q.bf_plane = best.ps;
    q.wcp = q.wtp;  q.wc_cs = q.wt_cs;  q.wc_bs = q.wt_bs;
  }
  if (best.lds > 64 * 1024) {
    static vsp::LdsAttrOnce raised[kMaxCfgs];
    if (int rc = raised[best.cfg].ensure(reinterpret_cast<const void*>(k.kern), (int)(k.PF == 3 ? kMaxLdsPipe : kMaxLds), "conv2d")) return rc;
  }
  q.wg_order = (q.dbg & 0x1000000) ? 0 : 1;
  if (k.PF == 3 && p.G == 1 && q.wg_order == 1 && !(q.dbg & 0x20000)) {
    const int64_t wtile = (int64_t)p.Cin * p.KH * p.KW * CO_T * 4, wall = wtile * best.co_tiles;
    const int64_t xall = (int64_t)p.B * p.Cin * p.H * p.W * 4;
    if (wall > 16 * 1024 * 1024 && best.co_tiles >= 4 && wall * 2 > xall / 8) {
      int cgs = (int)((int64_t)(2 * 1024 * 1024) / wtile);
      q.wg_cgs = cgs < 1 ? 1 : (cgs > best.co_tiles ? best.co_tiles : cgs);
      q.wg_order = 2;
    }
  }
  dim3 grid((unsigned)(best.tiles_x * best.tiles_y + (best.strip_col > 0 ? best.strip_col + best.strip_row : 0)), (unsigned)gy,
            (unsigned)p.B);
  dim3 block(64 * k.WM * k.WN * k.WK);
  hipLaunchKernelGGL(k.kern, grid, block, best.lds, vsp::as_stream(stream), q);
  return vsp::check_launch("conv2d");
}
```

### vspbfr_amd/csrc/conv_kernel.h

```cpp
#pragma once
#include "vsp_common.h"

namespace vspconv {

using f32x4 = __attribute__((ext_vector_type(4))) float;

struct ConvK {
  const float* x;
  const float* w;
  float* y;
  int B, Cin, H, W, G, cout_g, OH, OW, KH, KW, sy, sx;
  int dil[4], pady[4], padx[4];
  int y_ch, y_coff, y_h, y_w, osy, osx, ooy, oox;
  const float* in_scale;
  int in_scale_bstride;
  const float* in_shift;
  const float* osp; int oss;
  const float* csp; int css;
  const float* cbp; int cbs;
  const float* b1p; int b1s;
  float s1, g1;
  const float* nzp; int nzs;
  const float* nwp;
  const float* b2p; int b2s;
  const float* s2p; int s2s;
  float g2;
  const float* r1p; int r1s;
  const float* r2p; int r2s;
  int res_ch, res_coff;
  int tw_log2, th, tiles_x, tiles_y, co_tiles;
  int w_vec4;
  int ps_odd;
  int x_ch, x_gs;
  int strip_col;
  int dbg;
  int bf_pitch, bf_plane;
  int bf_isc_s, bf_ish_s;
  int wg_order;
  const float* wtp; int wt_cs, wt_bs;
  const float* wcp; int wc_cs, wc_bs;
  const float* wshp; int wsh_cs;
  int io_bf16;
  int64_t w_bs;
  int bf_tab;
  int wg_cgs;
  int rv_copad, rv_cbase, rv_ctot;
};

__device__ __forceinline__ int round_pitch(int n, int odd) {
  if (odd) return n | 1;
  int p = (n & ~31) + 16;
  return p >= n ? p : p + 32;
}

template <int MB, int NB, int WM, int WN, int CK, int WK, int PMAX, int PF, int OCC, bool TC = false, bool DG = false>
__global__ __launch_bounds__(64 * WM * WN * WK, OCC) void conv_igemm_kernel(const ConvK p) {
  static_assert(!TC || (NB % 4 == 0 && WK == 1), "transposed mode: N-blocks come in groups of four sub-pixel phases");
  constexpr int NP = TC ? NB / 4 : NB;
  static_assert(!DG || (MB == 4 && WM == 1 && WK == 1 && !TC), "dilation-group mode: M-block = group");
  constexpr int NT = 64 * WM * WN * WK;
  constexpr int CO_T = 16 * MB * WM;
  constexpr int WS = (CO_T % 32 == 0) ? CO_T + 16 : CO_T;
  extern __shared__ __attribute__((aligned(16))) float smem[];

  const int tid = threadIdx.x;
  const int lane = tid & 63;
  const int wave = __builtin_amdgcn_readfirstlane(tid >> 6);
  const int wk = wave / (WM * WN);
  const int wmn = wave - wk * (WM * WN);
  const int wm = wmn / WN, wn = wmn % WN;
  const int lr = lane & 15;
  const int kq = lane >> 4;

  int tile = blockIdx.x, by = blockIdx.y, bz = blockIdx.z;
  if (p.wg_order == 1) {
    const int GX = gridDim.x, GY = gridDim.y, GN = GX * GY, GT = GN * gridDim.z;
    const int wgid = blockIdx.x + GX * (blockIdx.y + GY * blockIdx.z);
    const int xcd = wgid & 7, xq = GT >> 3, xr = GT & 7;
    const int lid = (xcd < xr ? xcd * (xq + 1) : xr * (xq + 1) + (xcd - xr) * xq) + (wgid >> 3);
    bz = lid / GN;
    const int lrem = lid - bz * GN;
    tile = lrem / GY;
    by = lrem - tile * GY;
  }
  const int tx_i = tile % p.tiles_x, ty_i = tile / p.tiles_x;
  const int g = DG ? 0 : by / p.co_tiles;
  const int co0 = DG ? by * 16 : (by % p.co_tiles) * CO_T;
  const int b = bz;

  int twl = p.tw_log2, TH = p.th, oy0 = ty_i * p.th, ox0 = tx_i << p.tw_log2;
  int mlim = p.H + 1;
  if (TC && p.strip_col >= 0) {
    constexpr int NPIXB = 16 * WN * (NB / 4);
    mlim = p.H;
    int j = tile - p.tiles_x * p.tiles_y;
    if (j >= p.strip_col) {
      j -= p.strip_col;
      twl = __builtin_ctz(NPIXB); TH = 1; oy0 = p.H; ox0 = j * NPIXB; mlim = p.H + 1;
    } else if (j >= 0) {
      twl = 0; TH = NPIXB; oy0 = j * NPIXB; ox0 = p.W;
    }
  }
  const int TW = 1 << twl;
  const int gi = p.G > 4 ? 0 : g;
  const int D = DG ? max(max(p.dil[0], p.dil[1]), max(p.dil[2], p.dil[3])) : p.dil[gi];
  const int T = p.KH * p.KW;
  const int PH = TC ? TH + 1 : (TH - 1) * p.sy + (p.KH - 1) * D + 1;
  const int PW = TC ? TW + 1 : (TW - 1) * p.sx + (p.KW - 1) * D + 1;
  const int PS = round_pitch(PH * PW, p.ps_odd);
  const int iy0 = TC ? oy0 - 1 : DG ? oy0 - D : oy0 * p.sy - p.pady[gi];
  const int ix0 = TC ? ox0 - 1 : DG ? ox0 - D : ox0 * p.sx - p.padx[gi];

  float* Wl = smem;
  float* Pl = smem + T * CK * WS;

  int pixoff[NP];
#pragma unroll
  for (int nb = 0; nb < NP; ++nb) {
    const int n = (wn * NP + nb) * 16 + lr;
    const int py = n >> twl, px = n & (TW - 1);
    pixoff[nb] = py * p.sy * PW + px * p.sx + (kq + 4 * wk) * PS;
  }
  const int a_lane = (kq + 4 * wk) * WS + wm * MB * 16 + lr;

  f32x4 acc[MB][NB];
#pragma unroll
  for (int mb = 0; mb < MB; ++mb)
#pragma unroll
    for (int nb = 0; nb < NB; ++nb) acc[mb][nb] = f32x4{0.f, 0.f, 0.f, 0.f};

  const float* xb = p.x + ((int64_t)b * p.x_ch + (int64_t)g * p.x_gs) * p.H * p.W;
  const float* wg = p.w + (int64_t)g * T * p.Cin * p.cout_g;
  const __amdgpu_buffer_rsrc_t xrs = __builtin_amdgcn_make_buffer_rsrc(const_cast<float*>(xb), 0, 0x7fffffff, 0x00020000);
  const __amdgpu_buffer_rsrc_t wrs = __builtin_amdgcn_make_buffer_rsrc(const_cast<float*>(wg), 0, 0x7fffffff, 0x00020000);
  const int plane = PH * PW;
  const unsigned pw_magic = (unsigned)(((1ull << 32) + PW - 1) / PW);

  constexpr int NW = WM * WN * WK;
  constexpr int PCH = (CK + NW - 1) / NW;
  constexpr int V = CO_T / 4;
  constexpr int WMAX = (9 * CK * V + NT - 1) / NT;
  float4 wreg[WMAX];
  float preg[PF == 2 ? 1 : PCH][PF == 2 ? 1 : PMAX];
  float psc[PCH], psh[PCH];
  const int wtotal = T * CK * V;
  const int chw = p.H * p.W;

  auto patch_src = [&](int i, int& off) -> bool {
    const int r = (int)__umulhi((unsigned)i, pw_magic);
    const int c = i - r * PW;
    const int iy = iy0 + r, ix = ix0 + c;
    off = iy * p.W + ix;
    return iy >= 0 && iy < p.H && ix >= 0 && ix < p.W;
  };

  int poff[PMAX];
  unsigned pin = 0;
#pragma unroll
  for (int e = 0; e < PMAX; ++e) {
    const int i = lane + 64 * e;
    int off;
    const bool in = (i < plane) && patch_src(i, off);
    poff[e] = in ? off * 4 : 0;
    pin |= in ? (1u << e) : 0u;
  }
  int woff[WMAX];
  int wdst[WMAX];
#pragma unroll
  for (int w = 0; w < WMAX; ++w) {
    const int i = tid + w * NT;
    const int row = i / V, c4 = i - row * V;
    const int tap = row / CK, cl = row - tap * CK;
    const bool ok = i < wtotal;
    wdst[w] = ok ? row * WS + c4 * 4 : -1;
    if constexpr (DG) {
      const int cc = co0 + (c4 & 3) * 4;
      woff[w] = (ok && cc < p.cout_g) ? ((c4 >> 2) * T * p.Cin + tap * p.Cin + cl) * p.cout_g + cc : -1;
    } else {
      woff[w] = (ok && co0 + c4 * 4 < p.cout_g) ? (tap * p.Cin + cl) * p.cout_g + co0 + c4 * 4 : -1;
    }
  }

  auto issue = [&](int ci0) {
    if constexpr (PF == 2) return;
    if (p.w_vec4) {
      const int wsoff = ci0 * p.cout_g * 4;
#pragma unroll
      for (int w = 0; w < WMAX; ++w) {
        const int row = (tid + w * NT) / V;
        const int cl = row & (CK - 1);
        const bool ok = woff[w] >= 0 && ci0 + cl < p.Cin;
        const f32x4 v = __builtin_bit_cast(f32x4, __builtin_amdgcn_raw_buffer_load_b128(wrs, ok ? woff[w] * 4 : 0, wsoff, 0));
        wreg[w] = ok ? make_float4(v[0], v[1], v[2], v[3]) : make_float4(0.f, 0.f, 0.f, 0.f);
      }
    }
#pragma unroll
    for (int pc = 0; pc < PCH; ++pc) {
      const int cl = wave + pc * NW;
      const int ci = ci0 + cl;
      const bool chok = cl < CK && ci < p.Cin;
      const int cic = chok ? ci : 0;
      psc[pc] = chok ? (p.in_scale ? p.in_scale[(int64_t)b * p.in_scale_bstride + g * p.x_gs + cic] : 1.f) : 0.f;
      psh[pc] = chok ? (p.in_shift ? p.in_shift[cic] : 0.f) : 0.f;
      const int xsoff = cic * chw * 4;
#pragma unroll
      for (int e = 0; e < PMAX; ++e) preg[pc][e] = __builtin_bit_cast(float, __builtin_amdgcn_raw_buffer_load_b32(xrs, poff[e], xsoff, 0));
    }
  };

  auto commit = [&](int ci0) {
    if constexpr (PF == 2) return;
    if (p.w_vec4) {
#pragma unroll
      for (int w = 0; w < WMAX; ++w)
        if (wdst[w] >= 0) *reinterpret_cast<float4*>(Wl + wdst[w]) = wreg[w];
      for (int i = tid + WMAX * NT; i < wtotal; i += NT) {
        const int row = i / V, c4 = i - row * V;
        const int tap = row / CK, cl = row - tap * CK;
        const int ci = ci0 + cl;
        float4 v = make_float4(0.f, 0.f, 0.f, 0.f);
        if (ci < p.Cin && co0 + c4 * 4 < p.cout_g)
          v = *reinterpret_cast<const float4*>(wg + ((int64_t)tap * p.Cin + ci) * p.cout_g + co0 + c4 * 4);
        *reinterpret_cast<float4*>(Wl + row * WS + c4 * 4) = v;
      }
    } else {
#pragma unroll 4
      for (int i = tid; i < T * CK * CO_T; i += NT) {
        const int row = i / CO_T, c = i - row * CO_T;
        const int tap = row / CK, cl = row - tap * CK;
        const int ci = ci0 + cl;
        float v = 0.f;
        if (ci < p.Cin && co0 + c < p.cout_g) v = wg[((int64_t)tap * p.Cin + ci) * p.cout_g + co0 + c];
        Wl[row * WS + c] = v;
      }
    }
#pragma unroll
    for (int pc = 0; pc < PCH; ++pc) {
      const int cl = wave + pc * NW;
      if (cl >= CK) continue;
      const int ci = ci0 + cl;
      float* dst = Pl + cl * PS;
#pragma unroll
      for (int e = 0; e < PMAX; ++e) {
        const int i = lane + 64 * e;
        if (i < plane) dst[i] = ((pin >> e) & 1u) ? fmaf(preg[pc][e], psc[pc], psh[pc]) : 0.f;
      }
      if (plane > 64 * PMAX) {
        const bool chok = ci < p.Cin;
        const float* xc = xb + (int64_t)(chok ? ci : 0) * chw;
#pragma unroll 4
        for (int i0 = 64 * PMAX; i0 < plane; i0 += 64) {
          const int i = i0 + lane;
          int off;
          const bool in = patch_src(i < plane ? i : plane - 1, off) && chok && i < plane;
          const float xv = xc[in ? off : 0];
          if (i < plane) dst[i] = in ? fmaf(xv, psc[pc], psh[pc]) : 0.f;
        }
      }
    }
  };

  auto issue_async = [&](int ci0, float* Pdst) {
    const float* wc = wg + (int64_t)ci0 * p.cout_g;
#pragma unroll
    for (int w = 0; w < WMAX; ++w) {
      const int row = (tid + w * NT) / V;
      const int cl = row & (CK - 1);
      const bool ok = woff[w] >= 0 && ci0 + cl < p.Cin;
      const float4 v = *reinterpret_cast<const float4*>(wc + (ok ? woff[w] : 0));
      const float sc = (ok && p.in_scale) ? p.in_scale[(int64_t)b * p.in_scale_bstride + g * p.x_gs + ci0 + cl] : 1.f;
      wreg[w] = ok ? make_float4(v.x * sc, v.y * sc, v.z * sc, v.w * sc) : make_float4(0.f, 0.f, 0.f, 0.f);
    }
#pragma unroll
    for (int pc = 0; pc < PCH; ++pc) {
      const int cl = wave + pc * NW;
      const int ci = ci0 + cl;
      if (cl >= CK || ci >= p.Cin) continue;
      const float* xc = xb + (int64_t)ci * chw;
      float* dstc = Pdst + cl * PS;
#pragma unroll
      for (int e = 0; e < PMAX; ++e)
        if ((pin >> e) & 1u) __builtin_amdgcn_global_load_lds(xc + (poff[e] >> 2), dstc + 64 * e, 4, 0, 0);
      if (plane > 64 * PMAX) {
        for (int i0 = 64 * PMAX; i0 < plane; i0 += 64) {
          int off;
          if (i0 + lane < plane && patch_src(i0 + lane, off)) __builtin_amdgcn_global_load_lds(xc + off, dstc + i0, 4, 0, 0);
        }
      }
    }
  };
  auto commit_w = [&]() {
#pragma unroll
    for (int w = 0; w < WMAX; ++w)
      if (wdst[w] >= 0) *reinterpret_cast<float4*>(Wl + wdst[w]) = wreg[w];
  };
  if constexpr (PF == 2) {
    for (int i = tid; i < 2 * CK * PS; i += NT) Pl[i] = 0.f;
    __syncthreads();
    issue_async(0, Pl);
  } else if (PF) {
    issue(0);
  }
  int pbuf = 0;
  for (int ci0 = 0; ci0 < p.Cin; ci0 += CK) {
    __syncthreads();
    if constexpr (PF == 2) {
      commit_w();
    } else if (!(p.dbg & 1) || ci0 == 0) {
      if (!PF) issue(ci0);
      commit(ci0);
    }
    __syncthreads();
    if constexpr (PF == 2) {
      Pl = smem + T * CK * WS + pbuf * CK * PS;
      pbuf ^= 1;
      if (ci0 + CK < p.Cin) issue_async(ci0 + CK, smem + T * CK * WS + pbuf * CK * PS);
    } else {
      if (PF && ci0 + CK < p.Cin && !(p.dbg & 1)) issue(ci0 + CK);
    }
    if (p.dbg & 2) continue;
    if constexpr (TC) {
      constexpr int KS = CK / 4;
      float af[2][KS][MB], bf[2][KS][NP];
      auto load_tap = [&](int tap, float (&a)[KS][MB], float (&bq)[KS][NP]) {
        const int ky = tap / 3, kx = tap % 3;
        const int boff = (1 - (ky >> 1)) * PW + (1 - (kx >> 1));
        const float* wt = Wl + tap * CK * WS + a_lane;
#pragma unroll
        for (int c4 = 0; c4 < KS; ++c4) {
#pragma unroll
          for (int mb = 0; mb < MB; ++mb) a[c4][mb] = wt[c4 * 4 * WS + mb * 16];
#pragma unroll
          for (int np = 0; np < NP; ++np) bq[c4][np] = Pl[c4 * 4 * PS + pixoff[np] + boff];
        }
      };
      load_tap(0, af[0], bf[0]);
#pragma unroll
      for (int tap = 0; tap < 9; ++tap) {
        const int cur = tap & 1;
        if (tap < 8) load_tap(tap + 1, af[cur ^ 1], bf[cur ^ 1]);
        __builtin_amdgcn_sched_barrier(0);
        const int ph = ((tap / 3) & 1) * 2 + ((tap % 3) & 1);
#pragma unroll
        for (int c4 = 0; c4 < KS; ++c4)
#pragma unroll
          for (int mb = 0; mb < MB; ++mb)
#pragma unroll
            for (int np = 0; np < NP; ++np)
              acc[mb][np * 4 + ph] =
                  __builtin_amdgcn_mfma_f32_16x16x4f32(af[cur][c4][mb], bf[cur][c4][np], acc[mb][np * 4 + ph], 0, 0, 0);
        __builtin_amdgcn_sched_barrier(0);
      }
    } else if constexpr (DG) {
      int gbase[4];
#pragma unroll
      for (int gg = 0; gg < 4; ++gg) gbase[gg] = (D - p.dil[gg]) * (PW + 1);
      for (int ky = 0; ky < 3; ++ky) {
        for (int kx = 0; kx < 3; ++kx) {
          const float* wt = Wl + (ky * 3 + kx) * CK * WS + a_lane;
          int boff[4];
#pragma unroll
          for (int gg = 0; gg < 4; ++gg) boff[gg] = gbase[gg] + (ky * PW + kx) * p.dil[gg];
#pragma unroll
          for (int c4 = 0; c4 < CK / 4; ++c4) {
            float a[4];
#pragma unroll
            for (int gg = 0; gg < 4; ++gg) a[gg] = wt[c4 * 4 * WS + gg * 16];
#pragma unroll
            for (int gg = 0; gg < 4; ++gg) {
              float bv[NB];
#pragma unroll
              for (int nb = 0; nb < NB; ++nb) bv[nb] = Pl[c4 * 4 * PS + pixoff[nb] + boff[gg]];
#pragma unroll
              for (int nb = 0; nb < NB; ++nb)
                acc[gg][nb] = __builtin_amdgcn_mfma_f32_16x16x4f32(a[gg], bv[nb], acc[gg][nb], 0, 0, 0);
            }
          }
        }
      }
    } else {
      for (int ky = 0; ky < p.KH; ++ky) {
        for (int kx = 0; kx < p.KW; ++kx) {
          const int boff = ky * D * PW + kx * D;
          const float* wt = Wl + (ky * p.KW + kx) * CK * WS + a_lane;
#pragma unroll
          for (int c4 = 0; c4 < CK / 4; c4 += WK) {
            float a[MB], bv[NB];
#pragma unroll
            for (int mb = 0; mb < MB; ++mb) a[mb] = wt[c4 * 4 * WS + mb * 16];
#pragma unroll
            for (int nb = 0; nb < NB; ++nb) bv[nb] = Pl[c4 * 4 * PS + pixoff[nb] + boff];
#pragma unroll
            for (int mb = 0; mb < MB; ++mb)
#pragma unroll
              for (int nb = 0; nb < NB; ++nb)
                acc[mb][nb] = __builtin_amdgcn_mfma_f32_16x16x4f32(a[mb], bv[nb], acc[mb][nb], 0, 0, 0);
          }
        }
      }
    }
  }

  if (WK > 1) {
    __syncthreads();
    float* red = smem;
    if (wk > 0) {
#pragma unroll
      for (int mb = 0; mb < MB; ++mb)
#pragma unroll
        for (int nb = 0; nb < NB; ++nb)
#pragma unroll
          for (int r = 0; r < 4; ++r)
            red[((((wk - 1) * (WM * WN) + wmn) * (MB * NB * 4)) + (mb * NB + nb) * 4 + r) * 64 + lane] = acc[mb][nb][r];
    }
    __syncthreads();
    if (wk > 0) return;
#pragma unroll
    for (int k2 = 1; k2 < WK; ++k2)
#pragma unroll
      for (int mb = 0; mb < MB; ++mb)
#pragma unroll
        for (int nb = 0; nb < NB; ++nb)
#pragma unroll
          for (int r = 0; r < 4; ++r)
            acc[mb][nb][r] += red[((((k2 - 1) * (WM * WN) + wmn) * (MB * NB * 4)) + (mb * NB + nb) * 4 + r) * 64 + lane];
  }

  if (p.dbg & 4) return;
  const int Cout = p.G * p.cout_g;
  const float* osp = p.osp + (int64_t)b * Cout * p.oss;
  const float* nzp = p.nzp + (int64_t)b * p.OH * p.OW * p.nzs;
  const float nw = p.nwp[0];
  const float s1 = p.s1, g1 = p.g1, g2 = p.g2;
  const int oss = p.oss, css = p.css, cbs = p.cbs, b1s = p.b1s, b2s = p.b2s, s2s = p.s2s, nzs = p.nzs;

  float* yb = p.y + ((int64_t)b * p.y_ch + p.y_coff) * p.y_h * p.y_w;
  const float* r1b = p.r1p + ((int64_t)b * p.res_ch + p.res_coff) * p.y_h * p.y_w * p.r1s;
  const float* r2b = p.r2p + ((int64_t)b * p.res_ch + p.res_coff) * p.y_h * p.y_w * p.r2s;
  const int r1s = p.r1s, r2s = p.r2s;
  const int y_plane = p.y_h * p.y_w;

  if constexpr (TC) {
    typedef float f32x2u __attribute__((ext_vector_type(2), aligned(4)));
    int yoff[NP][2];
    bool pair[NP];
#pragma unroll
    for (int np = 0; np < NP; ++np) {
      const int n = (wn * NP + np) * 16 + lr;
      const int m = oy0 + (n >> twl), c = ox0 + (n & (TW - 1));
      const bool cok = c <= p.W;
      pair[np] = c < p.W;
#pragma unroll
      for (int py = 0; py < 2; ++py)
        yoff[np][py] = (cok && m < mlim && m < p.H + 1 - py) ? (2 * m + py) * p.y_w + 2 * c : -1;
    }
#pragma unroll
    for (int mb = 0; mb < MB; ++mb) {
#pragma unroll
      for (int r = 0; r < 4; ++r) {
        const int cg = co0 + (wm * MB + mb) * 16 + kq * 4 + r;
        const bool cok = cg < p.cout_g;
        const int co = cok ? cg : 0;
        const float os = osp[co * oss];
        const float cs = p.csp[co * css];
        const float cb = p.cbp[co * cbs];
        const float b1 = p.b1p[co * b1s];
        const float b2 = p.b2p[co * b2s];
        const float sl2 = p.s2p[co * s2s];
        float* yc = yb + (int64_t)co * y_plane;
        auto fin = [&](float v) {
          v = v * os * cs + cb + b1;
          v = (v > 0.f ? v : v * s1) * g1 + b2;
          return (v > 0.f ? v : v * sl2) * g2;
        };
#pragma unroll
        for (int np = 0; np < NP; ++np)
#pragma unroll
          for (int py = 0; py < 2; ++py) {
            if (yoff[np][py] < 0 || !cok) continue;
            const float v0 = fin(acc[mb][np * 4 + py * 2][r]), v1 = fin(acc[mb][np * 4 + py * 2 + 1][r]);
            if (pair[np])
              *reinterpret_cast<f32x2u*>(yc + yoff[np][py]) = f32x2u{v0, v1};
            else
              yc[yoff[np][py]] = v0;
          }
      }
    }
    return;
  }
  int yoff[NB];
  float nz[NB];
#pragma unroll
  for (int nb = 0; nb < NB; ++nb) {
    const int n = (wn * NB + nb) * 16 + lr;
    const int oy = oy0 + (n >> twl), ox = ox0 + (n & (TW - 1));
    const bool ok = (oy < p.OH && ox < p.OW);
    const int oyc = ok ? oy : 0, oxc = ok ? ox : 0;
    yoff[nb] = ok ? (oyc * p.osy + p.ooy) * p.y_w + oxc * p.osx + p.oox : -1;
    nz[nb] = nzp[(oyc * p.OW + oxc) * nzs] * nw;
  }
#pragma unroll
  for (int mb = 0; mb < MB; ++mb) {
#pragma unroll
    for (int r = 0; r < 4; ++r) {
      const int cg = DG ? co0 + kq * 4 + r : co0 + (wm * MB + mb) * 16 + kq * 4 + r;
      const bool cok = cg < p.cout_g;
      const int co = (DG ? mb : g) * p.cout_g + (cok ? cg : 0);
      const float os = osp[co * oss];
      const float cs = p.csp[co * css];
      const float cb = p.cbp[co * cbs];
      const float b1 = p.b1p[co * b1s];
      const float b2 = p.b2p[co * b2s];
      const float sl2 = p.s2p[co * s2s];
      const int cbase = co * y_plane;
#pragma unroll
      for (int nb = 0; nb < NB; ++nb) {
        const int ro = cbase + (yoff[nb] < 0 ? 0 : yoff[nb]);
        const float r1v = r1b[ro * r1s];
        const float r2v = r2b[ro * r2s];
        float v = acc[mb][nb][r] * os;
        v = v * cs + cb;
        v += b1;
        v = (v > 0.f ? v : v * s1) * g1;
        v += nz[nb];
        v += b2;
        v = (v > 0.f ? v : v * sl2) * g2;
        v += r1v;
        v += r2v;
        if (yoff[nb] >= 0 && cok) yb[ro] = v;
      }
    }
  }
}


int wino_launch(ConvK q, int form, hipStream_t stream);
bool smallmap_eligible(const ConvK& q, bool transposed);
int smallmap_launch(const ConvK& q, hipStream_t stream);
int wino_ro_launch(ConvK q, int mbw, int ivc, hipStream_t stream);
bool wino_ro_eligible(const ConvK& q);
int wino_rod_launch(ConvK q, int mbw, hipStream_t stream);
bool wino_rod_eligible(const ConvK& q);
int wino_rs_launch(ConvK q, hipStream_t stream);
bool wino_rs_eligible(const ConvK& q);
bool wino_rs_profitable(const ConvK& q);
inline bool quad_planes_ok(const ConvK& q, bool noise) {
  auto ok = [](const void* ptr, int stride) { return stride <= 1 && (!stride || vsp::aligned16(ptr)); };
  return vsp::aligned16(q.y) && ok(q.r1p, q.r1s) && ok(q.r2p, q.r2s) && (!noise || ok(q.nzp, q.nzs));
}
bool wino4_eligible(const ConvK& q);
size_t wino4_weight_floats(int cin, int cout);
size_t wino4_work_floats(int B, int cin, int H, int W);
int wino4_weight_launch(float* U, const float* wp, int cin, int cout, hipStream_t stream);
int wino4_launch(ConvK q, float* V, const float* scale, int scale_bs, hipStream_t stream);
bool wino4f_eligible(const ConvK& q);
size_t wino4f_weight_floats(int cin, int cout);
int wino4f_weight_launch(float* U, const float* wp, int cin, int cout, hipStream_t stream);
int wino4f_launch(ConvK q, hipStream_t stream);
int wino_chunk();
int wino_mbw(int cout_g);

int bf16_launch(const ConvK& q, int mode, int variant, hipStream_t stream);
int bf16_launch_split(const ConvK& q, int mode, int variant, hipStream_t stream);
bool bf16rv_eligible(const ConvK& q);
int bf16rv_launch(const ConvK& q, int variant, hipStream_t stream);
bool bf16dg_eligible(const ConvK& q);
int bf16dg_launch(const ConvK& q, bool full, hipStream_t stream);

struct Cfg {
  int MB, NB, WM, WN, CK, WK, PMAX, PF, OCC;
  const char* name;
  void (*kern)(const ConvK);
};

#define VSP_CFG(MB, NB, WM, WN, CK, WK, PMAX, PF, OCC)                                                     \
  {                                                                                                        \
    MB, NB, WM, WN, CK, WK, PMAX, PF, OCC, #MB "x" #NB "x" #WM "x" #WN "x" #CK "k" #WK "p" #PF "o" #OCC,  \
        conv_igemm_kernel<MB, NB, WM, WN, CK, WK, PMAX, PF, OCC>                                           \
  }

#define VSP_CFGM(MB, NB, WM, WN, CK, WK, PMAX, PF, OCC)                                                          \
  {                                                                                                              \
    MB, NB, WM, WN, CK, WK, PMAX, PF, OCC, #MB "x" #NB "x" #WM "x" #WN "x" #CK "k" #WK "p" #PF "o" #OCC "m" #PMAX, \
        conv_igemm_kernel<MB, NB, WM, WN, CK, WK, PMAX, PF, OCC>                                                 \
  }

#define VSP_CFGD(NB, WN, CK, PMAX, PF, OCC)                                                                \
  {                                                                                                        \
    4, NB, 1, WN, CK, 1, PMAX, PF, OCC, "4x" #NB "x1x" #WN "x" #CK "k1p" #PF "o" #OCC "d",                  \
        conv_igemm_kernel<4, NB, 1, WN, CK, 1, PMAX, PF, OCC, false, true>                                 \
  }

#define VSP_CFGT(MB, NB, WM, WN, CK, PMAX, PF, OCC)                                                        \
  {                                                                                                        \
    MB, NB, WM, WN, CK, 1, PMAX, PF, OCC, #MB "x" #NB "x" #WM "x" #WN "x" #CK "k1p" #PF "o" #OCC "t",       \
        conv_igemm_kernel<MB, NB, WM, WN, CK, 1, PMAX, PF, OCC, true>                                      \
  }

}
```

### vspbfr_amd/csrc/conv_pipe.hip

```cpp
#include "conv_kernel.h"
#include <type_traits>

#ifndef VSP_PIPE_SBU
#define VSP_PIPE_SBU 1
#endif
#ifndef VSP_PIPE_SBU_T
#define VSP_PIPE_SBU_T 1
#endif

namespace vspconv {

namespace {

__device__ __forceinline__ float uload(const float* base, int idx) {
  typedef const float __attribute__((address_space(4))) * cfp4;
  return ((cfp4)(uintptr_t)base)[__builtin_amdgcn_readfirstlane(idx)];
}

template <int MB, int NB, int WM, int WN, int CK, int PROWS, int OCC, int MODE, bool FG = false>
__global__ __launch_bounds__(64 * WM * WN, OCC) void conv_pipe_kernel(const ConvK p) {
  constexpr bool TC = MODE == 1, DG = MODE == 2, KG = MODE == 3, DGS = DG || KG;
  static_assert(!FG || DG, "fixed geometry serves the dilation-group mode");
  static_assert(!TC || NB % 4 == 0, "transposed mode: N-blocks come in groups of four sub-pixel phases");
  static_assert(!DGS || (MB == 4 && WM == 1), "dilation-group modes: M-block = group / block of 16 output channels");
  constexpr int NP = TC ? NB / 4 : NB;
  constexpr int NW = WM * WN, NT = 64 * NW;
  constexpr int CO_T = 16 * MB * WM;
  constexpr int WS = (CO_T % 32 == 0) ? CO_T + 16 : CO_T;
  constexpr int T = 9, KS = CK / 4, NU = T * KS;
  constexpr int F_NPOS = 16 * WN * NP;
  constexpr int F_TH = F_NPOS / 16;
  constexpr int F_PW = TC ? 17 : 32;
  constexpr int F_WPC = CK >= WM * WN ? 1 : WM * WN / CK;
  constexpr int F_PS = ((PROWS * F_WPC * 64) & ~31) + 16 >= PROWS * F_WPC * 64 ? ((PROWS * F_WPC * 64) & ~31) + 16
                                                                               : ((PROWS * F_WPC * 64) & ~31) + 48;
  constexpr int F_BUF = T * CK * WS + CK * F_PS;
  static_assert(!FG || !DG || F_TH == 16, "dilation-group fixed geometry: 16 x 16 pixels");
  extern __shared__ __attribute__((aligned(16))) float smem[];

  const int tid = threadIdx.x;
  const int lane = tid & 63;
  const int wave = __builtin_amdgcn_readfirstlane(tid >> 6);
  const int wm = wave / WN, wn = wave % WN;
  const int lr = lane & 15, kq = lane >> 4;

  int tile = blockIdx.x, by = blockIdx.y, bz = blockIdx.z;
  if (p.wg_order == 1) {
    const int GX = gridDim.x, GY = gridDim.y, GN = GX * GY, GT = GN * gridDim.z;
    const int wgid = blockIdx.x + GX * (blockIdx.y + GY * blockIdx.z);
    const int xcd = wgid & 7, xq = GT >> 3, xr = GT & 7;
    const int lid = (xcd < xr ? xcd * (xq + 1) : xr * (xq + 1) + (xcd - xr) * xq) + (wgid >> 3);
    bz = lid / GN;
    const int lrem = lid - bz * GN;
    tile = lrem / GY;
    by = lrem - tile * GY;
  } else if (p.wg_order == 2) {
    const int GX = gridDim.x, GY = gridDim.y, GT = GX * GY * gridDim.z;
    const int wgid = blockIdx.x + GX * (blockIdx.y + GY * blockIdx.z);
    const int xcd = wgid & 7, xq = GT >> 3, xr = GT & 7;
    const int lid = (xcd < xr ? xcd * (xq + 1) : xr * (xq + 1) + (xcd - xr) * xq) + (wgid >> 3);
    const int cgs = p.wg_cgs, npt = GX * (int)gridDim.z;
    const int full = (GY / cgs) * cgs * npt;
    int cgrp, rem, cw;
    if (lid < full) { cgrp = lid / (cgs * npt); rem = lid - cgrp * (cgs * npt); cw = cgs; }
    else { cgrp = GY / cgs; rem = lid - full; cw = GY - cgrp * cgs; }
    const int pt = rem / cw;
    by = cgrp * cgs + (rem - pt * cw);
    bz = pt / GX;
    tile = pt - bz * GX;
  }
  const int tx_i = tile % p.tiles_x, ty_i = tile / p.tiles_x;
  const int g = DGS ? 0 : by / p.co_tiles;
  const int co0 = DGS ? by * 16 : (by % p.co_tiles) * CO_T;
  const int b = bz;
  int twl = FG ? 4 : p.tw_log2, TH = FG ? F_TH : p.th, oy0 = ty_i * (FG ? F_TH : p.th), ox0 = tx_i << (FG ? 4 : p.tw_log2);
  int mlim = p.H + 1;
  if (TC && !FG && p.strip_col >= 0) {
    constexpr int NPIXB = 16 * WN * NP;
    mlim = p.H;
    int j = tile - p.tiles_x * p.tiles_y;
    if (j >= p.strip_col) {
      j -= p.strip_col;
      twl = __builtin_ctz(NPIXB); TH = 1; oy0 = p.H; ox0 = j * NPIXB; mlim = p.H + 1;
    } else if (j >= 0) {
      twl = 0; TH = NPIXB; oy0 = j * NPIXB; ox0 = p.W;
    }
  }
  const int TW = 1 << twl;
  const int gi = p.G > 4 ? 0 : g;
  const int D = DGS ? max(max(p.dil[0], p.dil[1]), max(p.dil[2], p.dil[3])) : p.dil[gi];
  const int PH = TC ? TH + 1 : (TH - 1) * p.sy + 2 * D + 1;
  const int PW = FG ? F_PW : TC ? TW + 1 : (TW - 1) * p.sx + 2 * D + 1;
  const int plane = PH * PW;
  const int PS = FG ? F_PS : p.bf_plane;
  const int BUF = FG ? F_BUF : T * CK * WS + CK * PS;
  const int iy0 = TC ? oy0 - 1 : DGS ? oy0 - D : oy0 * p.sy - p.pady[gi];
  const int ix0 = TC ? ox0 - 1 : DGS ? ox0 - D : ox0 * p.sx - p.padx[gi];

  int pixoff[NP];
#pragma unroll
  for (int nb = 0; nb < NP; ++nb) {
    const int n = (wn * NP + nb) * 16 + lr;
    const int py = n >> twl, px = n & (TW - 1);
    pixoff[nb] = T * CK * WS + py * p.sy * PW + px * p.sx + kq * PS;
  }
  const int a_lane = kq * WS + wm * MB * 16 + lr;

  f32x4 acc[MB][NB];
#pragma unroll
  for (int mb = 0; mb < MB; ++mb)
#pragma unroll
    for (int nb = 0; nb < NB; ++nb) acc[mb][nb] = f32x4{0.f, 0.f, 0.f, 0.f};

  const int chw = p.H * p.W;
  const float* xb = p.x + ((int64_t)b * p.x_ch + (int64_t)g * p.x_gs) * chw;
  const float* wg = p.w + (int64_t)g * T * p.Cin * p.cout_g;
  constexpr int kOOB = 0x7ffffff0;
  const __amdgpu_buffer_rsrc_t xrs =
      __builtin_amdgcn_make_buffer_rsrc(const_cast<float*>(xb), 0, (p.x_ch - g * p.x_gs) * chw * 4, 0x00020000);
  const __amdgpu_buffer_rsrc_t wrs = __builtin_amdgcn_make_buffer_rsrc(const_cast<float*>(wg), 0, (DGS ? 4 : 1) * T * p.Cin * p.cout_g * 4, 0x00020000);
  const unsigned pw_magic = (unsigned)(((1ull << 32) + PW - 1) / PW);

  constexpr int PCH = CK >= NW ? CK / NW : 1;
  constexpr int WPC = CK >= NW ? 1 : NW / CK;
  const int pcl0 = CK >= NW ? wave : wave / WPC;
  const int j0 = CK >= NW ? 0 : wave % WPC;
  int poff[PROWS];
#pragma unroll
  for (int e = 0; e < PROWS; ++e) {
    const int i = (j0 + WPC * e) * 64 + lane;
    const int r = (int)__umulhi((unsigned)i, pw_magic);
    const int c = i - r * PW;
    const int iy = iy0 + r, ix = ix0 + c;
    const bool in = i < plane && iy >= 0 && iy < p.H && ix >= 0 && ix < p.W;
    poff[e] = in ? (iy * p.W + ix) * 4 : kOOB;
  }
  const int pdst = T * CK * WS + pcl0 * PS + j0 * 64 + lane;
  constexpr int V = CO_T / 4;
  constexpr int WITEMS = T * CK * V;
  constexpr int WF = WITEMS / NT;
  constexpr int RV = ((WITEMS % NT) * 4 + NT - 1) / NT;
  static_assert(RV <= 2, "weight tail must split into at most 2 floats per thread");
  static_assert(RV == 0 || (WS > CO_T && NT / 16 <= T * CK), "tail threads without a piece need the slab's pad columns");
  constexpr int WMAX = WF + (RV ? 1 : 0);
  int woff[WMAX];
  int wdst[WMAX];
#pragma unroll
  for (int w = 0; w < WMAX; ++w) {
    const int f = w < WF ? (tid + w * NT) * 4 : WF * NT * 4 + tid * RV;
    const int i = f >> 2, sub = f & 3;
    const int row = i / V, c4 = i - row * V;
    const int tap = row / CK, cl = row - tap * CK;
    const bool piece = i < WITEMS;
    wdst[w] = piece ? row * WS + c4 * 4 + sub
                    : (RV == 2 ? ((tid >> 3) % (T * CK)) * WS + CO_T + (tid & 7) * 2 : (tid >> 4) * WS + CO_T + (tid & 15));
    if constexpr (DGS) {
      const int cc = co0 + (c4 & 3) * 4 + sub;
      woff[w] = (piece && cc < p.cout_g) ? (((c4 >> 2) * T * p.Cin + tap * p.Cin + cl) * p.cout_g + cc) * 4 : kOOB;
    } else {
      const int cc = co0 + c4 * 4 + sub;
      woff[w] = (piece && cc < p.cout_g) ? ((tap * p.Cin + cl) * p.cout_g + cc) * 4 : kOOB;
    }
  }
  f32x4 wreg[WMAX];
  float preg[PCH][PROWS];
  float psc[PCH];

  constexpr int NITEM = WMAX + PCH * PROWS;
  auto issue_item = [&](int k, int ci0) {
    if (k < WF) {
      wreg[k] = __builtin_bit_cast(f32x4, __builtin_amdgcn_raw_buffer_load_b128(wrs, woff[k], ci0 * p.cout_g * 4, 0));
    } else if (k < WMAX) {
      if constexpr (RV == 2) {
        typedef float f32x2 __attribute__((ext_vector_type(2)));
        const f32x2 v = __builtin_bit_cast(f32x2, __builtin_amdgcn_raw_buffer_load_b64(wrs, woff[k], ci0 * p.cout_g * 4, 0));
        wreg[k][0] = v[0]; wreg[k][1] = v[1];
      } else {
        wreg[k][0] = __builtin_bit_cast(float, __builtin_amdgcn_raw_buffer_load_b32(wrs, woff[k], ci0 * p.cout_g * 4, 0));
      }
    } else {
      const int pc = (k - WMAX) / PROWS, e = (k - WMAX) % PROWS;
      const int ci = ci0 + pcl0 + pc * NW;
      preg[pc][e] = __builtin_bit_cast(float, __builtin_amdgcn_raw_buffer_load_b32(xrs, poff[e], ci * chw * 4, 0));
    }
  };
  auto load_scales = [&](int ci0) {
#pragma unroll
    for (int pc = 0; pc < PCH; ++pc)
      psc[pc] = uload(p.wcp, b * p.wc_bs + (g * p.x_gs + ci0 + pcl0 + pc * NW) * p.wc_cs);
  };
  auto commit_item = [&](int k, float* buf) {
    if (k < WF) {
      *reinterpret_cast<f32x4*>(buf + wdst[k]) = wreg[k];
    } else if (k < WMAX) {
      if constexpr (RV == 2) {
        typedef float f32x2 __attribute__((ext_vector_type(2)));
        *reinterpret_cast<f32x2*>(buf + wdst[k]) = f32x2{wreg[k][0], wreg[k][1]};
      } else {
        buf[wdst[k]] = wreg[k][0];
      }
    } else {
      const int pc = (k - WMAX) / PROWS, e = (k - WMAX) % PROWS;
      buf[pdst + pc * NW * PS + e * (WPC * 64)] = preg[pc][e] * psc[pc];
    }
  };

  float af[2][MB], bfr[2][NP];
  int kg_d = D, kg_b = 0;
  auto load_frag = [&](int u, const float* buf, float (&a)[MB], float (&bq)[NP]) {
    const int tap = u / KS, c4 = u % KS;
    const int ky = tap / 3, kx = tap % 3;
    const float* wt = buf + (tap * CK + c4 * 4) * WS + a_lane;
#pragma unroll
    for (int mb = 0; mb < MB; ++mb) a[mb] = wt[mb * 16];
    if constexpr (!DG) {
      const int boff = TC ? (1 - (ky >> 1)) * PW + (1 - (kx >> 1)) : KG ? kg_b + (ky * PW + kx) * kg_d : (ky * PW + kx) * D;
#pragma unroll
      for (int np = 0; np < NP; ++np) bq[np] = buf[c4 * 4 * PS + pixoff[np] + boff];
    }
  };
  auto mfma_unit = [&](int u, const float (&a)[MB], const float (&bq)[NP]) {
    const int tap = u / KS;
    if constexpr (TC) {
      const int ph = ((tap / 3) & 1) * 2 + ((tap % 3) & 1);
#pragma unroll
      for (int mb = 0; mb < MB; ++mb)
#pragma unroll
        for (int np = 0; np < NP; ++np)
          acc[mb][np * 4 + ph] = __builtin_amdgcn_mfma_f32_16x16x4f32(a[mb], bq[np], acc[mb][np * 4 + ph], 0, 0, 0);
    } else {
#pragma unroll
      for (int mb = 0; mb < MB; ++mb)
#pragma unroll
        for (int nb = 0; nb < NB; ++nb)
          acc[mb][nb] = __builtin_amdgcn_mfma_f32_16x16x4f32(a[mb], bq[nb], acc[mb][nb], 0, 0, 0);
    }
  };
  int gbase[4];
  if constexpr (DG) {
#pragma unroll
    for (int gg = 0; gg < 4; ++gg) gbase[gg] = (D - p.dil[gg]) * (PW + 1);
  }
  float bdg[2][4][NB];
  auto load_frag_dg = [&](int u, const float* buf, float (&a)[MB], float (&bq)[4][NB]) {
    const int tap = u / KS, c4 = u % KS;
    const int ky = tap / 3, kx = tap % 3;
    const float* wt = buf + (tap * CK + c4 * 4) * WS + a_lane;
#pragma unroll
    for (int gg = 0; gg < 4; ++gg) a[gg] = wt[gg * 16];
#pragma unroll
    for (int gg = 0; gg < 4; ++gg) {
      const int boff = gbase[gg] + (ky * PW + kx) * p.dil[gg];
#pragma unroll
      for (int nb = 0; nb < NB; ++nb) bq[gg][nb] = buf[c4 * 4 * PS + pixoff[nb] + boff];
    }
  };
  auto mfma_unit_dg = [&](const float (&a)[MB], const float (&bq)[4][NB]) {
#pragma unroll
    for (int gg = 0; gg < 4; ++gg)
#pragma unroll
      for (int nb = 0; nb < NB; ++nb) acc[gg][nb] = __builtin_amdgcn_mfma_f32_16x16x4f32(a[gg], bq[gg][nb], acc[gg][nb], 0, 0, 0);
  };

  const int nchunk = (p.Cin + CK - 1) / CK;
  constexpr int NUI = NU >= 6 ? NU / 3 : 1;
  constexpr int NUC = NU - NUI;
  constexpr int SBU = TC ? VSP_PIPE_SBU_T : VSP_PIPE_SBU;
  auto interval = [&](int i, auto commit_tag, auto issue_tag) {
    constexpr bool COMMIT = decltype(commit_tag)::value, ISSUE = decltype(issue_tag)::value;
    const float* cur = smem + (i & 1) * BUF;
    float* nxt = smem + ((i + 1) & 1) * BUF;
    if constexpr (COMMIT) load_scales((i + 1) * CK);
    if constexpr (KG) {
      const int q4 = p.Cin >> 2, ci = i * CK;
      kg_d = ci < q4 ? p.dil[0] : ci < 2 * q4 ? p.dil[1] : ci < 3 * q4 ? p.dil[2] : p.dil[3];
      kg_b = (D - kg_d) * (PW + 1);
    }
    if constexpr (DG) load_frag_dg(0, cur, af[0], bdg[0]); else load_frag(0, cur, af[0], bfr[0]);
#pragma unroll
    for (int u = 0; u < NU; ++u) {
      const int s = u & 1;
      if (u + 1 < NU) {
        if constexpr (DG) load_frag_dg(u + 1, cur, af[s ^ 1], bdg[s ^ 1]); else load_frag(u + 1, cur, af[s ^ 1], bfr[s ^ 1]);
      }
      if constexpr (DG) mfma_unit_dg(af[s], bdg[s]); else mfma_unit(u, af[s], bfr[s]);
      if (COMMIT && u < NUC) {
#pragma unroll
        for (int k = u * NITEM / NUC; k < (u + 1) * NITEM / NUC; ++k) commit_item(k, nxt);
      }
      if (ISSUE && u >= NUC) {
#pragma unroll
        for (int k = (u - NUC) * NITEM / NUI; k < (u - NUC + 1) * NITEM / NUI; ++k) issue_item(k, (i + 2) * CK);
      }
      if ((u + 1) % SBU == 0 || u + 1 == NU) __builtin_amdgcn_sched_barrier(0);
    }
    __syncthreads();
  };
  {
#pragma unroll
    for (int k = 0; k < NITEM; ++k) issue_item(k, 0);
    load_scales(0);
#pragma unroll
    for (int k = 0; k < NITEM; ++k) commit_item(k, smem);
    if (nchunk > 1) {
#pragma unroll
      for (int k = 0; k < NITEM; ++k) issue_item(k, CK);
    }
    __syncthreads();
  }
  if constexpr (!FG) {
    int iv = 0;
    for (; iv < nchunk - 2; ++iv) interval(iv, std::true_type{}, std::true_type{});
    if (nchunk >= 2) { interval(iv, std::true_type{}, std::false_type{}); ++iv; }
    interval(iv, std::false_type{}, std::false_type{});
  } else {
    const int fa = a_lane;
    const int fb = T * CK * WS + (wn * NP) * F_PW + lr + kq * F_PS;
    constexpr int NS = T * KS;
    constexpr int NSI = NS >= 6 ? NS / 3 : 1, NSC = NS - NSI;
    auto staging = [&](int sidx, int i, auto commit_tag, auto issue_tag, float* nxt) {
      constexpr bool COMMIT = decltype(commit_tag)::value, ISSUE = decltype(issue_tag)::value;
      if (COMMIT && sidx < NSC) {
#pragma unroll
        for (int k = sidx * NITEM / NSC; k < (sidx + 1) * NITEM / NSC; ++k) commit_item(k, nxt);
      }
      if (ISSUE && sidx >= NSC) {
#pragma unroll
        for (int k = (sidx - NSC) * NITEM / NSI; k < (sidx - NSC + 1) * NITEM / NSI; ++k) issue_item(k, (i + 2) * CK);
      }
      __builtin_amdgcn_sched_barrier(0);
    };
    {
      float ga[2][4], gb[2][4][NB];
      auto load_dg = [&](int u, int cur, float (&a)[4], float (&b)[4][NB]) {
        const int tap = u / KS, c4 = u % KS;
        const int ky = tap / 3, kx = tap % 3;
#pragma unroll
        for (int gg = 0; gg < 4; ++gg) a[gg] = smem[fa + cur + (tap * CK + c4 * 4) * WS + gg * 16];
#pragma unroll
        for (int gg = 0; gg < 4; ++gg) {
          const int d_ = 1 << gg;
          const int off = (8 - d_) * (F_PW + 1) + (ky * F_PW + kx) * d_;
#pragma unroll
          for (int nb = 0; nb < NB; ++nb) b[gg][nb] = smem[fb + cur + c4 * 4 * F_PS + nb * F_PW + off];
        }
      };
      auto interval_fg = [&](int i, auto par_tag, auto commit_tag, auto issue_tag) {
        constexpr int PAR = decltype(par_tag)::value;
        constexpr bool COMMIT = decltype(commit_tag)::value;
        constexpr int cur = PAR * F_BUF, nxo = (1 - PAR) * F_BUF;
        if constexpr (COMMIT) load_scales((i + 1) * CK);
        load_dg(0, cur, ga[0], gb[0]);
#pragma unroll
        for (int u = 0; u < NS; ++u) {
          const int s_ = u & 1;
          if (u + 1 < NS) load_dg(u + 1, cur, ga[s_ ^ 1], gb[s_ ^ 1]);
#pragma unroll
          for (int gg = 0; gg < 4; ++gg)
#pragma unroll
            for (int nb = 0; nb < NB; ++nb)
              acc[gg][nb] = __builtin_amdgcn_mfma_f32_16x16x4f32(ga[s_][gg], gb[s_][gg][nb], acc[gg][nb], 0, 0, 0);
          staging(u, i, commit_tag, issue_tag, smem + nxo);
        }
        __syncthreads();
      };
      int iv = 0;
      for (; iv + 3 < nchunk; iv += 2) {
        interval_fg(iv, std::integral_constant<int, 0>{}, std::true_type{}, std::true_type{});
        interval_fg(iv + 1, std::integral_constant<int, 1>{}, std::true_type{}, std::true_type{});
      }
      for (; iv < nchunk; ++iv) {
        const bool c_ = iv + 1 < nchunk, s2 = iv + 2 < nchunk;
        if (iv & 1) {
          if (s2) interval_fg(iv, std::integral_constant<int, 1>{}, std::true_type{}, std::true_type{});
          else if (c_) interval_fg(iv, std::integral_constant<int, 1>{}, std::true_type{}, std::false_type{});
          else interval_fg(iv, std::integral_constant<int, 1>{}, std::false_type{}, std::false_type{});
        } else {
          if (s2) interval_fg(iv, std::integral_constant<int, 0>{}, std::true_type{}, std::true_type{});
          else if (c_) interval_fg(iv, std::integral_constant<int, 0>{}, std::true_type{}, std::false_type{});
          else interval_fg(iv, std::integral_constant<int, 0>{}, std::false_type{}, std::false_type{});
        }
      }
    }
  }

  const int Cout = p.G * p.cout_g;
  const float* osp = p.osp + (int64_t)b * Cout * p.oss;
  const float s1 = p.s1, g1 = p.g1, g2 = p.g2;
  const int oss = p.oss, css = p.css, cbs = p.cbs, b1s = p.b1s, b2s = p.b2s, s2s = p.s2s;
  float* yb = p.y + ((int64_t)b * p.y_ch + p.y_coff) * p.y_h * p.y_w;
  const int y_plane = p.y_h * p.y_w;
  if constexpr (TC) {
    typedef float f32x2u __attribute__((ext_vector_type(2), aligned(4)));
    int yoff[NP][2];
    bool pair[NP];
#pragma unroll
    for (int np = 0; np < NP; ++np) {
      const int n = (wn * NP + np) * 16 + lr;
      const int m = oy0 + (n >> twl), c = ox0 + (n & (TW - 1));
      const bool cok = c <= p.W;
      pair[np] = c < p.W;
#pragma unroll
      for (int py = 0; py < 2; ++py)
        yoff[np][py] = (cok && m < mlim && m < p.H + 1 - py) ? (2 * m + py) * p.y_w + 2 * c : -1;
    }
    const bool only_os = css == 0 && cbs == 0 && b1s == 0 && b2s == 0 && s2s == 0 && s1 == 1.f && g1 == 1.f && g2 == 1.f &&
                         __builtin_amdgcn_readfirstlane(__builtin_bit_cast(int, p.s2p[0])) == 0x3f800000;
    if (only_os) {
#pragma unroll
      for (int mb = 0; mb < MB; ++mb) {
#pragma unroll
        for (int r = 0; r < 4; ++r) {
          const int cg = co0 + (wm * MB + mb) * 16 + kq * 4 + r;
          const bool cok = cg < p.cout_g;
          const int co = cok ? cg : 0;
          const float os = osp[co * oss];
          float* yc = yb + (int64_t)co * y_plane;
#pragma unroll
          for (int np = 0; np < NP; ++np)
#pragma unroll
            for (int py = 0; py < 2; ++py) {
              if (yoff[np][py] < 0 || !cok) continue;
              const float v0 = acc[mb][np * 4 + py * 2][r] * os, v1 = acc[mb][np * 4 + py * 2 + 1][r] * os;
              if (pair[np])
                *reinterpret_cast<f32x2u*>(yc + yoff[np][py]) = f32x2u{v0, v1};
              else
                yc[yoff[np][py]] = v0;
            }
        }
      }
      return;
    }
#pragma unroll
    for (int mb = 0; mb < MB; ++mb) {
#pragma unroll
      for (int r = 0; r < 4; ++r) {
        const int cg = co0 + (wm * MB + mb) * 16 + kq * 4 + r;
        const bool cok = cg < p.cout_g;
        const int co = cok ? cg : 0;
        const float os = osp[co * oss], cs = p.csp[co * css], cb = p.cbp[co * cbs];
        const float b1 = p.b1p[co * b1s], b2 = p.b2p[co * b2s], sl2 = p.s2p[co * s2s];
        float* yc = yb + (int64_t)co * y_plane;
        auto fin = [&](float v) {
          v = v * os * cs + cb + b1;
          v = (v > 0.f ? v : v * s1) * g1 + b2;
          return (v > 0.f ? v : v * sl2) * g2;
        };
#pragma unroll
        for (int np = 0; np < NP; ++np)
#pragma unroll
          for (int py = 0; py < 2; ++py) {
            if (yoff[np][py] < 0 || !cok) continue;
            const float v0 = fin(acc[mb][np * 4 + py * 2][r]), v1 = fin(acc[mb][np * 4 + py * 2 + 1][r]);
            if (pair[np])
              *reinterpret_cast<f32x2u*>(yc + yoff[np][py]) = f32x2u{v0, v1};
            else
              yc[yoff[np][py]] = v0;
          }
      }
    }
    return;
  } else {
    const float* nzp = p.nzp + (int64_t)b * p.OH * p.OW * p.nzs;
    const float nw = p.nwp[0];
    const int nzs = p.nzs;
    const float* r1b = p.r1p + ((int64_t)b * p.res_ch + p.res_coff) * p.y_h * p.y_w * p.r1s;
    const float* r2b = p.r2p + ((int64_t)b * p.res_ch + p.res_coff) * p.y_h * p.y_w * p.r2s;
    const int r1s = p.r1s, r2s = p.r2s;
    int yoff[NB];
    float nz[NB];
#pragma unroll
    for (int nb = 0; nb < NB; ++nb) {
      const int n = (wn * NB + nb) * 16 + lr;
      const int oy = oy0 + (n >> twl), ox = ox0 + (n & (TW - 1));
      const bool ok = (oy < p.OH && ox < p.OW);
      const int oyc = ok ? oy : 0, oxc = ok ? ox : 0;
      yoff[nb] = ok ? (oyc * p.osy + p.ooy) * p.y_w + oxc * p.osx + p.oox : -1;
      nz[nb] = nzp[(oyc * p.OW + oxc) * nzs] * nw;
    }
#pragma unroll
    for (int mb = 0; mb < MB; ++mb) {
#pragma unroll
      for (int r = 0; r < 4; ++r) {
        const int cg = DGS ? co0 + kq * 4 + r : co0 + (wm * MB + mb) * 16 + kq * 4 + r;
        const bool cok = cg < p.cout_g;
        const int co = (DGS ? mb : g) * p.cout_g + (cok ? cg : 0);
        const float os = osp[co * oss], cs = p.csp[co * css], cb = p.cbp[co * cbs];
        const float b1 = p.b1p[co * b1s], b2 = p.b2p[co * b2s], sl2 = p.s2p[co * s2s];
        const int cbase = co * y_plane;
#pragma unroll
        for (int nb = 0; nb < NB; ++nb) {
          const int ro = cbase + (yoff[nb] < 0 ? 0 : yoff[nb]);
          const float r1v = r1b[ro * r1s];
          const float r2v = r2b[ro * r2s];
          float v = acc[mb][nb][r] * os;
          v = v * cs + cb;
          v += b1;
          v = (v > 0.f ? v : v * s1) * g1;
          v += nz[nb];
          v += b2;
          v = (v > 0.f ? v : v * sl2) * g2;
          v += r1v;
          v += r2v;
          if (yoff[nb] >= 0 && cok) yb[ro] = v;
        }
      }
    }
  }
}

}

#define VSP_CFGP(MB, NB, WM, WN, CK, PROWS, OCC)                                                     \
  {                                                                                                  \
    MB, NB, WM, WN, CK, 1, PROWS, 3, OCC, #MB "x" #NB "x" #WM "x" #WN "x" #CK "k1p3o" #OCC "r" #PROWS, \
        conv_pipe_kernel<MB, NB, WM, WN, CK, PROWS, OCC, 0>                                          \
  }
#define VSP_CFGPT(MB, NB, WM, WN, CK, PROWS, OCC)                                                    \
  {                                                                                                  \
    MB, NB, WM, WN, CK, 1, PROWS, 3, OCC, #MB "x" #NB "x" #WM "x" #WN "x" #CK "k1p3o" #OCC "r" #PROWS "t", \
        conv_pipe_kernel<MB, NB, WM, WN, CK, PROWS, OCC, 1>                                          \
  }
#define VSP_CFGPD(NB, WN, CK, PROWS, OCC)                                                            \
  {                                                                                                  \
    4, NB, 1, WN, CK, 1, PROWS, 3, OCC, "4x" #NB "x1x" #WN "x" #CK "k1p3o" #OCC "r" #PROWS "d",        \
        conv_pipe_kernel<4, NB, 1, WN, CK, PROWS, OCC, 2>                                            \
  }

#define VSP_CFGPDF(NB, WN, CK, PROWS, OCC)                                                           \
  {                                                                                                  \
    4, NB, 1, WN, CK, 1, PROWS, 3, OCC, "4x" #NB "x1x" #WN "x" #CK "k1p3o" #OCC "r" #PROWS "fd",       \
        conv_pipe_kernel<4, NB, 1, WN, CK, PROWS, OCC, 2, true>                                      \
  }

#define VSP_CFGPK(NB, WN, CK, PROWS, OCC)                                                            \
  {                                                                                                  \
    4, NB, 1, WN, CK, 1, PROWS, 3, OCC, "4x" #NB "x1x" #WN "x" #CK "k1p3o" #OCC "r" #PROWS "a",        \
        conv_pipe_kernel<4, NB, 1, WN, CK, PROWS, OCC, 3>                                            \
  }

extern const Cfg kCfgsP[] = {
    VSP_CFGP(4, 4, 2, 4, 8, 18, 1),
    VSP_CFGP(4, 2, 2, 4, 8, 9, 1),
    VSP_CFGP(4, 4, 2, 4, 4, 9, 1),
    VSP_CFGP(4, 4, 1, 4, 8, 9, 1),
    VSP_CFGP(4, 2, 2, 4, 4, 5, 1),
    VSP_CFGP(2, 4, 2, 4, 8, 18, 1),
    VSP_CFGP(2, 4, 2, 4, 4, 9, 1),
    VSP_CFGP(4, 4, 1, 8, 8, 18, 1),
    VSP_CFGP(4, 2, 2, 4, 4, 5, 2),
    VSP_CFGP(2, 4, 2, 4, 4, 9, 2),
    VSP_CFGP(2, 2, 2, 4, 8, 9, 2),
    VSP_CFGP(2, 2, 2, 4, 4, 5, 2),
    VSP_CFGPT(2, 16, 2, 4, 8, 9, 1),
    VSP_CFGPT(2, 16, 2, 4, 4, 5, 1),
    VSP_CFGPT(2, 8, 2, 4, 8, 5, 1),
    VSP_CFGPT(4, 8, 2, 4, 8, 5, 1),
    VSP_CFGPT(1, 16, 2, 4, 8, 9, 1),
    VSP_CFGPT(2, 8, 2, 4, 8, 5, 2),
    VSP_CFGPT(2, 8, 2, 4, 4, 3, 2),
    VSP_CFGPT(1, 8, 2, 4, 8, 5, 2),
    VSP_CFGPT(2, 8, 1, 4, 8, 3, 2),
    VSP_CFGPD(2, 8, 4, 8, 2),
    VSP_CFGPD(2, 8, 8, 16, 1),
    VSP_CFGPD(4, 4, 4, 16, 1),
    VSP_CFGPD(4, 4, 8, 16, 1),
    VSP_CFGPD(4, 8, 4, 12, 1),
    VSP_CFGPDF(2, 8, 4, 8, 4),
    VSP_CFGPDF(2, 8, 4, 8, 2),
    VSP_CFGPDF(2, 8, 8, 16, 1),
    VSP_CFGPK(2, 8, 4, 8, 2),
    VSP_CFGPK(2, 8, 8, 16, 1),
    VSP_CFGPK(4, 8, 4, 12, 1),
    VSP_CFGPK(4, 4, 4, 16, 1),
};
extern const int kNumP = sizeof(kCfgsP) / sizeof(kCfgsP[0]);

}
```

Baseline: 204.9 img/s.

## Make pipelined conv kernel walk flattened work items with cross-item prefetch

Turns the pipelined implicit-GEMM conv kernel into a grid-stride walker over a flattened 1D list of work items, decoded from virtual grid dimensions passed as kernel arguments. It can prefetch the next item's first input chunks while the current item finishes and runs its epilogue. Per-item setup (buffer resources, pixel offsets, scale bases) moves into lambdas that are re-run per item, with sched barriers and asm fences added to limit register pressure. The grid size comes from an occupancy-based slot count or an env override. By default it equals the item count, so each workgroup still handles one item and mainly pays the extra decode and reload overhead.

Result: no change. 205.3 img/s (median of 6 runs) (+0.2%).

```diff
diff --git a/include/vspbfr_hip.h b/include/vspbfr_hip.h
--- a/include/vspbfr_hip.h
+++ b/include/vspbfr_hip.h
@@ -105,6 +105,7 @@
 int vsp_winograd_weight_f32(float* U, const float* wp, int G, int cin, int cout_g, vsp_stream_t stream);
 int vsp_conv2d_num_configs(void);
 const char* vsp_conv2d_config_name(int i);
+int vsp_conv2d_pipe_grid(int64_t items, int slots, int wgs);
 
 int vsp_conv2d_bf16(const vsp_conv_params* p, vsp_stream_t stream);
 
diff --git a/vspbfr_amd/_lib.py b/vspbfr_amd/_lib.py
--- a/vspbfr_amd/_lib.py
+++ b/vspbfr_amd/_lib.py
@@ -121,6 +121,7 @@
     "vsp_upfirdn2d_f32": [_p, _p, _p] + [_i] * 14 + [C.POINTER(FirEpilogue), _p],
     "vsp_conv2d_f32": [C.POINTER(ConvParams), _p],
     "vsp_conv2d_num_configs": [],
+    "vsp_conv2d_pipe_grid": [_i64, _i, _i],
     "vsp_gemm_f32": [C.POINTER(GemmParams), _p],
     "vsp_pixelnorm_dim1_f32": [_p, _p, _i, _i, _i, _f, _p],
     "vsp_layernorm_f32": [_p, _p, _p, _p, _p, _i, _i, _f, _i, _f, _f, _p],
diff --git a/vspbfr_amd/csrc/conv_igemm.hip b/vspbfr_amd/csrc/conv_igemm.hip
--- a/vspbfr_amd/csrc/conv_igemm.hip
+++ b/vspbfr_amd/csrc/conv_igemm.hip
@@ -346,6 +346,33 @@
   return VSP_OK;
 }
 
+extern "C" int vsp_conv2d_pipe_grid(int64_t items, int slots, int wgs) {
+  if (items < 1) return 0;
+  int64_t g = wgs == 0 ? items : wgs > 0 ? wgs : slots;
+  if (g < 1) g = 1;
+  if (g > items) g = items;
+  return (int)(g > 0x7fffffff ? 0x7fffffff : g);
+}
+
+static int pipe_slots(int cfg, int odd, const void* fn, int block, size_t lds, int* out) {
+  constexpr int kDevs = 16;
+  static std::atomic<int> cache[kMaxCfgs][2][kDevs];
+  int dev = 0;
+  if (hipGetDevice(&dev) != hipSuccess || dev < 0) return vsp::fail(VSP_ELAUNCH, "conv2d: hipGetDevice failed");
+  std::atomic<int>* slot = dev < kDevs ? &cache[cfg][odd ? 1 : 0][dev] : nullptr;
+  int v = slot ? slot->load(std::memory_order_acquire) : 0;
+  if (v <= 0) {
+    int per_cu = 0, cus = 0;
+    hipError_t e = hipOccupancyMaxActiveBlocksPerMultiprocessor(&per_cu, fn, block, lds);
+    if (e == hipSuccess) e = hipDeviceGetAttribute(&cus, hipDeviceAttributeMultiprocessorCount, dev);
+    if (e != hipSuccess) return vsp::fail(VSP_ELAUNCH, "conv2d: occupancy query failed: %s", hipGetErrorString(e));
+    v = (per_cu < 1 ? 1 : per_cu) * (cus < 1 ? vsp::kNumCU : cus);
+    if (slot) slot->store(v, std::memory_order_release);
+  }
+  *out = v;
+  return VSP_OK;
+}
+
 extern "C" int vsp_conv2d_num_configs(void) {
   build_table();
   return kNumCfgs + 1;
@@ -596,6 +623,19 @@
   dim3 grid((unsigned)(best.tiles_x * best.tiles_y + (best.strip_col > 0 ? best.strip_col + best.strip_row : 0)), (unsigned)gy,
             (unsigned)p.B);
   dim3 block(64 * k.WM * k.WN * k.WK);
+  const CfgKind kind = cfg_kind(k);
+  if (k.PF == 3 && !kind.dg && !kind.kg) {
+    const int64_t items = (int64_t)grid.x * grid.y * grid.z;
+    VSP_REQUIRE(items < ((int64_t)1 << 30), "conv2d: too many work items (%lld)", (long long)items);
+    static const int wgs_env = vsp::tune_env("VSP_PIPE_WGS") ? atoi(vsp::tune_env("VSP_PIPE_WGS")) : -2;
+    const int wgs = wgs_env != -2 ? wgs_env : 0;
+    int slots = 0;
+    if (wgs < 0)
+      if (int rc = pipe_slots(best.cfg, q.ps_odd, reinterpret_cast<const void*>(k.kern), (int)block.x, best.lds, &slots)) return rc;
+    q.vg_x = (int)grid.x; q.vg_y = (int)grid.y; q.vg_z = (int)grid.z;
+    q.n_items = (int)items;
+    grid = dim3((unsigned)vsp_conv2d_pipe_grid(items, slots, wgs), 1, 1);
+  }
   hipLaunchKernelGGL(k.kern, grid, block, best.lds, vsp::as_stream(stream), q);
   return vsp::check_launch("conv2d");
 }
diff --git a/vspbfr_amd/csrc/conv_kernel.h b/vspbfr_amd/csrc/conv_kernel.h
--- a/vspbfr_amd/csrc/conv_kernel.h
+++ b/vspbfr_amd/csrc/conv_kernel.h
@@ -44,6 +44,7 @@
   int64_t w_bs;
   int bf_tab;
   int wg_cgs;
+  int vg_x, vg_y, vg_z, n_items;
   int rv_copad, rv_cbase, rv_ctot;
 };
 
diff --git a/vspbfr_amd/csrc/conv_pipe.hip b/vspbfr_amd/csrc/conv_pipe.hip
--- a/vspbfr_amd/csrc/conv_pipe.hip
+++ b/vspbfr_amd/csrc/conv_pipe.hip
@@ -16,6 +16,43 @@
   typedef const float __attribute__((address_space(4))) * cfp4;
   return ((cfp4)(uintptr_t)base)[__builtin_amdgcn_readfirstlane(idx)];
 }
+
+__device__ __forceinline__ void pipe_decode(const ConvK& p, int v, int GX, int GY, int GZ, int& tile, int& by, int& bz) {
+  if (p.wg_order == 0) {
+    tile = v % GX;
+    const int t = v / GX;
+    by = t % GY;
+    bz = t / GY;
+    return;
+  }
+  const int GN = GX * GY, GT = GN * GZ;
+  const int xcd = v & 7, xq = GT >> 3, xr = GT & 7;
+  const int lid = (xcd < xr ? xcd * (xq + 1) : xr * (xq + 1) + (xcd - xr) * xq) + (v >> 3);
+  if (p.wg_order == 1) {
+    bz = lid / GN;
+    const int lrem = lid - bz * GN;
+    tile = lrem / GY;
+    by = lrem - tile * GY;
+  } else {
+    const int cgs = p.wg_cgs, npt = GX * GZ;
+    const int full = (GY / cgs) * cgs * npt;
+    int cgrp, rem, cw;
+    if (lid < full) { cgrp = lid / (cgs * npt); rem = lid - cgrp * (cgs * npt); cw = cgs; }
+    else { cgrp = GY / cgs; rem = lid - full; cw = GY - cgrp * cgs; }
+    const int pt = rem / cw;
+    by = cgrp * cgs + (rem - pt * cw);
+    bz = pt / GX;
+    tile = pt - bz * GX;
+  }
+}
+
+struct PipeItem {
+  int oy0, ox0, ck, gb;
+  __device__ __forceinline__ int co0() const { return ck & ~3; }
+  __device__ __forceinline__ int kind() const { return ck & 3; }
+  __device__ __forceinline__ int g() const { return gb & 0xffff; }
+  __device__ __forceinline__ int b() const { return (int)((unsigned)gb >> 16); }
+};
 
 template <int MB, int NB, int WM, int WN, int CK, int PROWS, int OCC, int MODE, bool FG = false>
 __global__ __launch_bounds__(64 * WM * WN, OCC) void conv_pipe_kernel(const ConvK p) {
@@ -41,101 +78,102 @@
   const int tid = threadIdx.x;
   const int lane = tid & 63;
   const int wave = __builtin_amdgcn_readfirstlane(tid >> 6);
-  const int wm = wave / WN, wn = wave % WN;
+  const int wn = wave % WN;
   const int lr = lane & 15, kq = lane >> 4;
 
-  int tile = blockIdx.x, by = blockIdx.y, bz = blockIdx.z;
-  if (p.wg_order == 1) {
-    const int GX = gridDim.x, GY = gridDim.y, GN = GX * GY, GT = GN * gridDim.z;
-    const int wgid = blockIdx.x + GX * (blockIdx.y + GY * blockIdx.z);
-    const int xcd = wgid & 7, xq = GT >> 3, xr = GT & 7;
-    const int lid = (xcd < xr ? xcd * (xq + 1) : xr * (xq + 1) + (xcd - xr) * xq) + (wgid >> 3);
-    bz = lid / GN;
-    const int lrem = lid - bz * GN;
-    tile = lrem / GY;
-    by = lrem - tile * GY;
-  } else if (p.wg_order == 2) {
-    const int GX = gridDim.x, GY = gridDim.y, GT = GX * GY * gridDim.z;
-    const int wgid = blockIdx.x + GX * (blockIdx.y + GY * blockIdx.z);
-    const int xcd = wgid & 7, xq = GT >> 3, xr = GT & 7;
-    const int lid = (xcd < xr ? xcd * (xq + 1) : xr * (xq + 1) + (xcd - xr) * xq) + (wgid >> 3);
-    const int cgs = p.wg_cgs, npt = GX * (int)gridDim.z;
-    const int full = (GY / cgs) * cgs * npt;
-    int cgrp, rem, cw;
-    if (lid < full) { cgrp = lid / (cgs * npt); rem = lid - cgrp * (cgs * npt); cw = cgs; }
-    else { cgrp = GY / cgs; rem = lid - full; cw = GY - cgrp * cgs; }
-    const int pt = rem / cw;
-    by = cgrp * cgs + (rem - pt * cw);
-    bz = pt / GX;
-    tile = pt - bz * GX;
-  }
-  const int tx_i = tile % p.tiles_x, ty_i = tile / p.tiles_x;
-  const int g = DGS ? 0 : by / p.co_tiles;
-  const int co0 = DGS ? by * 16 : (by % p.co_tiles) * CO_T;
-  const int b = bz;
-  int twl = FG ? 4 : p.tw_log2, TH = FG ? F_TH : p.th, oy0 = ty_i * (FG ? F_TH : p.th), ox0 = tx_i << (FG ? 4 : p.tw_log2);
-  int mlim = p.H + 1;
-  if (TC && !FG && p.strip_col >= 0) {
-    constexpr int NPIXB = 16 * WN * NP;
-    mlim = p.H;
-    int j = tile - p.tiles_x * p.tiles_y;
-    if (j >= p.strip_col) {
-      j -= p.strip_col;
-      twl = __builtin_ctz(NPIXB); TH = 1; oy0 = p.H; ox0 = j * NPIXB; mlim = p.H + 1;
-    } else if (j >= 0) {
-      twl = 0; TH = NPIXB; oy0 = j * NPIXB; ox0 = p.W;
-    }
-  }
-  const int TW = 1 << twl;
-  const int gi = p.G > 4 ? 0 : g;
-  const int D = DGS ? max(max(p.dil[0], p.dil[1]), max(p.dil[2], p.dil[3])) : p.dil[gi];
-  const int PH = TC ? TH + 1 : (TH - 1) * p.sy + 2 * D + 1;
-  const int PW = FG ? F_PW : TC ? TW + 1 : (TW - 1) * p.sx + 2 * D + 1;
-  const int plane = PH * PW;
+  constexpr bool WALK = (MODE == 0 || MODE == 1) && !FG;
+  constexpr int NPIXB = 16 * WN * NP;
+  auto kargs = [&]() -> const ConvK& {
+    if constexpr (WALK) {
+      typedef const ConvK __attribute__((address_space(4))) * ckp4;
+      ckp4 q = (ckp4)__builtin_amdgcn_kernarg_segment_ptr();
+      asm volatile("" : "+s"(q));
+      return *(const ConvK*)q;
+    } else {
+      return p;
+    }
+  };
+  auto fresh_v = [](int v) {
+    if constexpr (WALK) asm volatile("" : "+v"(v));
+    return v;
+  };
+  auto fresh_s = [](int v) {
+    if constexpr (WALK) asm volatile("" : "+s"(v));
+    return v;
+  };
+  auto make_item = [&](int v) __attribute__((always_inline)) {
+    const ConvK& p = kargs();
+    const int GX = WALK ? p.vg_x : (int)gridDim.x, GY = WALK ? p.vg_y : (int)gridDim.y, GZ = WALK ? p.vg_z : (int)gridDim.z;
+    int tile, by, bz;
+    pipe_decode(p, v, GX, GY, GZ, tile, by, bz);
+    PipeItem it;
+    const int ty_i = tile / p.tiles_x, tx_i = tile - ty_i * p.tiles_x;
+    const int g_ = DGS ? 0 : by / p.co_tiles;
+    it.gb = g_ | (bz << 16);
+    it.ck = DGS ? by * 16 : (by - g_ * p.co_tiles) * CO_T;
+    it.oy0 = ty_i * (FG ? F_TH : p.th);
+    it.ox0 = tx_i << (FG ? 4 : p.tw_log2);
+    if (TC && !FG && p.strip_col >= 0) {
+      int j = tile - p.tiles_x * p.tiles_y;
+      if (j >= p.strip_col) {
+        j -= p.strip_col;
+        it.ck |= 2; it.oy0 = p.H; it.ox0 = j * NPIXB;
+      } else if (j >= 0) {
+        it.ck |= 1; it.oy0 = j * NPIXB; it.ox0 = p.W;
+      }
+    }
+    it.oy0 = __builtin_amdgcn_readfirstlane(it.oy0); it.ox0 = __builtin_amdgcn_readfirstlane(it.ox0);
+    it.ck = __builtin_amdgcn_readfirstlane(it.ck); it.gb = __builtin_amdgcn_readfirstlane(it.gb);
+    return it;
+  };
+  auto kind_twl = [&](int kind) { const ConvK& p = kargs(); return FG ? 4 : (!TC || kind == 0) ? p.tw_log2 : kind == 1 ? 0 : __builtin_ctz(NPIXB); };
+  auto kind_th = [&](int kind) { const ConvK& p = kargs(); return FG ? F_TH : (!TC || kind == 0) ? p.th : kind == 1 ? NPIXB : 1; };
+  auto item_dil = [&](int g_) { const ConvK& p = kargs(); return DGS ? max(max(p.dil[0], p.dil[1]), max(p.dil[2], p.dil[3])) : p.dil[p.G > 4 ? 0 : g_]; };
+
+  int D, PW;
   const int PS = FG ? F_PS : p.bf_plane;
   const int BUF = FG ? F_BUF : T * CK * WS + CK * PS;
-  const int iy0 = TC ? oy0 - 1 : DGS ? oy0 - D : oy0 * p.sy - p.pady[gi];
-  const int ix0 = TC ? ox0 - 1 : DGS ? ox0 - D : ox0 * p.sx - p.padx[gi];
-
-  int pixoff[NP];
-#pragma unroll
-  for (int nb = 0; nb < NP; ++nb) {
-    const int n = (wn * NP + nb) * 16 + lr;
-    const int py = n >> twl, px = n & (TW - 1);
-    pixoff[nb] = T * CK * WS + py * p.sy * PW + px * p.sx + kq * PS;
-  }
-  const int a_lane = kq * WS + wm * MB * 16 + lr;
+  int pixoff[NP], a_lane;
+  auto set_mult = [&](const PipeItem& it) __attribute__((always_inline)) {
+    const ConvK& p = kargs();
+    const int lane_f = fresh_v((int)threadIdx.x) & 63, wave_f = fresh_s(wave);
+    const int lr = lane_f & 15, kq = lane_f >> 4, wn = wave_f % WN;
+    const int twl = kind_twl(it.kind()), TW = 1 << twl;
+    D = item_dil(it.g());
+    PW = FG ? F_PW : TC ? TW + 1 : (TW - 1) * p.sx + 2 * D + 1;
+#pragma unroll
+    for (int nb = 0; nb < NP; ++nb) {
+      const int n = (wn * NP + nb) * 16 + lr;
+      const int py = n >> twl, px = n & (TW - 1);
+      pixoff[nb] = T * CK * WS + py * p.sy * PW + px * p.sx + kq * PS;
+    }
+    a_lane = kq * WS + (wave_f / WN) * MB * 16 + lr;
+  };
 
   f32x4 acc[MB][NB];
-#pragma unroll
-  for (int mb = 0; mb < MB; ++mb)
-#pragma unroll
-    for (int nb = 0; nb < NB; ++nb) acc[mb][nb] = f32x4{0.f, 0.f, 0.f, 0.f};
+  auto clear_acc = [&]() __attribute__((always_inline)) {
+    float z = 0.f;
+    if constexpr (WALK) asm volatile("" : "+v"(z));
+#pragma unroll
+    for (int mb = 0; mb < MB; ++mb)
+#pragma unroll
+      for (int nb = 0; nb < NB; ++nb) acc[mb][nb] = f32x4{z, z, z, z};
+  };
+  clear_acc();
 
   const int chw = p.H * p.W;
-  const float* xb = p.x + ((int64_t)b * p.x_ch + (int64_t)g * p.x_gs) * chw;
-  const float* wg = p.w + (int64_t)g * T * p.Cin * p.cout_g;
   constexpr int kOOB = 0x7ffffff0;
-  const __amdgpu_buffer_rsrc_t xrs =
-      __builtin_amdgcn_make_buffer_rsrc(const_cast<float*>(xb), 0, (p.x_ch - g * p.x_gs) * chw * 4, 0x00020000);
-  const __amdgpu_buffer_rsrc_t wrs = __builtin_amdgcn_make_buffer_rsrc(const_cast<float*>(wg), 0, (DGS ? 4 : 1) * T * p.Cin * p.cout_g * 4, 0x00020000);
-  const unsigned pw_magic = (unsigned)(((1ull << 32) + PW - 1) / PW);
+  __amdgpu_buffer_rsrc_t xrs = __builtin_amdgcn_make_buffer_rsrc(const_cast<float*>(p.x), 0, 0, 0x00020000);
+  __amdgpu_buffer_rsrc_t wrs = __builtin_amdgcn_make_buffer_rsrc(const_cast<float*>(p.w), 0, 0, 0x00020000);
+  int i_pw = 0;
+  unsigned pw_magic = 0;
+  int i_sbase = 0;
 
   constexpr int PCH = CK >= NW ? CK / NW : 1;
   constexpr int WPC = CK >= NW ? 1 : NW / CK;
   const int pcl0 = CK >= NW ? wave : wave / WPC;
-  const int j0 = CK >= NW ? 0 : wave % WPC;
   int poff[PROWS];
-#pragma unroll
-  for (int e = 0; e < PROWS; ++e) {
-    const int i = (j0 + WPC * e) * 64 + lane;
-    const int r = (int)__umulhi((unsigned)i, pw_magic);
-    const int c = i - r * PW;
-    const int iy = iy0 + r, ix = ix0 + c;
-    const bool in = i < plane && iy >= 0 && iy < p.H && ix >= 0 && ix < p.W;
-    poff[e] = in ? (iy * p.W + ix) * 4 : kOOB;
-  }
-  const int pdst = T * CK * WS + pcl0 * PS + j0 * 64 + lane;
+  int pdst;
   constexpr int V = CO_T / 4;
   constexpr int WITEMS = T * CK * V;
   constexpr int WF = WITEMS / NT;
@@ -145,23 +183,74 @@
   constexpr int WMAX = WF + (RV ? 1 : 0);
   int woff[WMAX];
   int wdst[WMAX];
-#pragma unroll
-  for (int w = 0; w < WMAX; ++w) {
-    const int f = w < WF ? (tid + w * NT) * 4 : WF * NT * 4 + tid * RV;
-    const int i = f >> 2, sub = f & 3;
-    const int row = i / V, c4 = i - row * V;
-    const int tap = row / CK, cl = row - tap * CK;
-    const bool piece = i < WITEMS;
-    wdst[w] = piece ? row * WS + c4 * 4 + sub
-                    : (RV == 2 ? ((tid >> 3) % (T * CK)) * WS + CO_T + (tid & 7) * 2 : (tid >> 4) * WS + CO_T + (tid & 15));
-    if constexpr (DGS) {
-      const int cc = co0 + (c4 & 3) * 4 + sub;
-      woff[w] = (piece && cc < p.cout_g) ? (((c4 >> 2) * T * p.Cin + tap * p.Cin + cl) * p.cout_g + cc) * 4 : kOOB;
-    } else {
-      const int cc = co0 + c4 * 4 + sub;
-      woff[w] = (piece && cc < p.cout_g) ? ((tap * p.Cin + cl) * p.cout_g + cc) * 4 : kOOB;
-    }
-  }
+  auto set_dst = [&]() __attribute__((always_inline)) {
+    const int tid = fresh_v((int)threadIdx.x), lane = tid & 63;
+    const int wave_f = fresh_s(wave);
+    const int pcl0 = CK >= NW ? wave_f : wave_f / WPC, j0 = CK >= NW ? 0 : wave_f % WPC;
+    pdst = T * CK * WS + pcl0 * PS + j0 * 64 + lane;
+#pragma unroll
+    for (int w = 0; w < WMAX; ++w) {
+      const int f = w < WF ? (tid + w * NT) * 4 : WF * NT * 4 + tid * RV;
+      const int i = f >> 2, sub = f & 3;
+      const int row = i / V, c4 = i - row * V;
+      const bool piece = i < WITEMS;
+      wdst[w] = piece ? row * WS + c4 * 4 + sub
+                      : (RV == 2 ? ((tid >> 3) % (T * CK)) * WS + CO_T + (tid & 7) * 2 : (tid >> 4) * WS + CO_T + (tid & 15));
+    }
+  };
+  set_dst();
+  auto plan_issue = [&](const PipeItem& it) __attribute__((always_inline)) {
+    const ConvK& p = kargs();
+    const int tid = fresh_v((int)threadIdx.x), lane = tid & 63;
+    const int wave_f = fresh_s(wave);
+    const int pcl0 = CK >= NW ? wave_f : wave_f / WPC, j0 = CK >= NW ? 0 : wave_f % WPC;
+    const int twl_ = kind_twl(it.kind()), TW_ = 1 << twl_, TH_ = kind_th(it.kind()), D_ = item_dil(it.g());
+    const int gi = p.G > 4 ? 0 : it.g();
+    const int PH_ = TC ? TH_ + 1 : (TH_ - 1) * p.sy + 2 * D_ + 1;
+    const int PW_ = FG ? F_PW : TC ? TW_ + 1 : (TW_ - 1) * p.sx + 2 * D_ + 1;
+    const int plane = PH_ * PW_;
+    const int iy0 = TC ? it.oy0 - 1 : DGS ? it.oy0 - D_ : it.oy0 * p.sy - p.pady[gi];
+    const int ix0 = TC ? it.ox0 - 1 : DGS ? it.ox0 - D_ : it.ox0 * p.sx - p.padx[gi];
+    if (PW_ != i_pw) {
+      i_pw = PW_;
+      pw_magic = (unsigned)(((1ull << 32) + PW_ - 1) / PW_);
+    }
+    const float* xb = p.x + ((int64_t)it.b() * p.x_ch + (int64_t)it.g() * p.x_gs) * chw;
+    const float* wg = p.w + (int64_t)it.g() * T * p.Cin * p.cout_g;
+    xrs = __builtin_amdgcn_make_buffer_rsrc(const_cast<float*>(xb), 0, (p.x_ch - it.g() * p.x_gs) * chw * 4, 0x00020000);
+    wrs = __builtin_amdgcn_make_buffer_rsrc(const_cast<float*>(wg), 0, (DGS ? 4 : 1) * T * p.Cin * p.cout_g * 4, 0x00020000);
+    i_sbase = it.b() * p.wc_bs + (it.g() * p.x_gs + pcl0) * p.wc_cs;
+#pragma unroll
+    for (int e = 0; e < PROWS; ++e) {
+      const int i = (j0 + WPC * e) * 64 + lane;
+      const int r = (int)__umulhi((unsigned)i, pw_magic);
+      const int c = i - r * PW_;
+      const int iy = iy0 + r, ix = ix0 + c;
+      const bool in = i < plane && iy >= 0 && iy < p.H && ix >= 0 && ix < p.W;
+      poff[e] = in ? (iy * p.W + ix) * 4 : kOOB;
+      if constexpr (WALK) __builtin_amdgcn_sched_barrier(0);
+    }
+#pragma unroll
+    for (int w = 0; w < WMAX; ++w) {
+      const int f = w < WF ? (tid + w * NT) * 4 : WF * NT * 4 + tid * RV;
+      const int i = f >> 2, sub = f & 3;
+      const int row = i / V, c4 = i - row * V;
+      const int tap = row / CK, cl = row - tap * CK;
+      const bool piece = i < WITEMS;
+      if constexpr (DGS) {
+        const int cc = it.co0() + (c4 & 3) * 4 + sub;
+        woff[w] = (piece && cc < p.cout_g) ? (((c4 >> 2) * T * p.Cin + tap * p.Cin + cl) * p.cout_g + cc) * 4 : kOOB;
+      } else {
+        const int cc = it.co0() + c4 * 4 + sub;
+        woff[w] = (piece && cc < p.cout_g) ? ((tap * p.Cin + cl) * p.cout_g + cc) * 4 : kOOB;
+      }
+      if constexpr (WALK) __builtin_amdgcn_sched_barrier(0);
+    }
+  };
+  const int v0 = WALK ? (int)blockIdx.x : (int)(blockIdx.x + gridDim.x * (blockIdx.y + gridDim.y * blockIdx.z));
+  PipeItem item = make_item(v0);
+  set_mult(item);
+  plan_issue(item);
   f32x4 wreg[WMAX];
   float preg[PCH][PROWS];
   float psc[PCH];
@@ -184,10 +273,9 @@
       preg[pc][e] = __builtin_bit_cast(float, __builtin_amdgcn_raw_buffer_load_b32(xrs, poff[e], ci * chw * 4, 0));
     }
   };
-  auto load_scales = [&](int ci0) {
-#pragma unroll
-    for (int pc = 0; pc < PCH; ++pc)
-      psc[pc] = uload(p.wcp, b * p.wc_bs + (g * p.x_gs + ci0 + pcl0 + pc * NW) * p.wc_cs);
+  auto load_scales = [&](int si) {
+#pragma unroll
+    for (int pc = 0; pc < PCH; ++pc) psc[pc] = uload(p.wcp, si + pc * NW * p.wc_cs);
   };
   auto commit_item = [&](int k, float* buf) {
     if (k < WF) {
@@ -206,7 +294,7 @@
   };
 
   float af[2][MB], bfr[2][NP];
-  int kg_d = D, kg_b = 0;
+  int kg_d = 1, kg_b = 0;
   auto load_frag = [&](int u, const float* buf, float (&a)[MB], float (&bq)[NP]) {
     const int tap = u / KS, c4 = u % KS;
     const int ky = tap / 3, kx = tap % 3;
@@ -266,11 +354,11 @@
   constexpr int NUI = NU >= 6 ? NU / 3 : 1;
   constexpr int NUC = NU - NUI;
   constexpr int SBU = TC ? VSP_PIPE_SBU_T : VSP_PIPE_SBU;
-  auto interval = [&](int i, auto commit_tag, auto issue_tag) {
+  auto interval = [&](int i, int si, int ci2, auto commit_tag, auto issue_tag) {
     constexpr bool COMMIT = decltype(commit_tag)::value, ISSUE = decltype(issue_tag)::value;
     const float* cur = smem + (i & 1) * BUF;
     float* nxt = smem + ((i + 1) & 1) * BUF;
-    if constexpr (COMMIT) load_scales((i + 1) * CK);
+    if constexpr (COMMIT) load_scales(si);
     if constexpr (KG) {
       const int q4 = p.Cin >> 2, ci = i * CK;
       kg_d = ci < q4 ? p.dil[0] : ci < 2 * q4 ? p.dil[1] : ci < 3 * q4 ? p.dil[2] : p.dil[3];
@@ -290,100 +378,19 @@
       }
       if (ISSUE && u >= NUC) {
 #pragma unroll
-        for (int k = (u - NUC) * NITEM / NUI; k < (u - NUC + 1) * NITEM / NUI; ++k) issue_item(k, (i + 2) * CK);
+        for (int k = (u - NUC) * NITEM / NUI; k < (u - NUC + 1) * NITEM / NUI; ++k) issue_item(k, ci2);
       }
       if ((u + 1) % SBU == 0 || u + 1 == NU) __builtin_amdgcn_sched_barrier(0);
     }
     __syncthreads();
   };
-  {
-#pragma unroll
-    for (int k = 0; k < NITEM; ++k) issue_item(k, 0);
-    load_scales(0);
-#pragma unroll
-    for (int k = 0; k < NITEM; ++k) commit_item(k, smem);
-    if (nchunk > 1) {
-#pragma unroll
-      for (int k = 0; k < NITEM; ++k) issue_item(k, CK);
-    }
-    __syncthreads();
-  }
-  if constexpr (!FG) {
-    int iv = 0;
-    for (; iv < nchunk - 2; ++iv) interval(iv, std::true_type{}, std::true_type{});
-    if (nchunk >= 2) { interval(iv, std::true_type{}, std::false_type{}); ++iv; }
-    interval(iv, std::false_type{}, std::false_type{});
-  } else {
-    const int fa = a_lane;
-    const int fb = T * CK * WS + (wn * NP) * F_PW + lr + kq * F_PS;
-    constexpr int NS = T * KS;
-    constexpr int NSI = NS >= 6 ? NS / 3 : 1, NSC = NS - NSI;
-    auto staging = [&](int sidx, int i, auto commit_tag, auto issue_tag, float* nxt) {
-      constexpr bool COMMIT = decltype(commit_tag)::value, ISSUE = decltype(issue_tag)::value;
-      if (COMMIT && sidx < NSC) {
-#pragma unroll
-        for (int k = sidx * NITEM / NSC; k < (sidx + 1) * NITEM / NSC; ++k) commit_item(k, nxt);
-      }
-      if (ISSUE && sidx >= NSC) {
-#pragma unroll
-        for (int k = (sidx - NSC) * NITEM / NSI; k < (sidx - NSC + 1) * NITEM / NSI; ++k) issue_item(k, (i + 2) * CK);
-      }
-      __builtin_amdgcn_sched_barrier(0);
-    };
-    {
-      float ga[2][4], gb[2][4][NB];
-      auto load_dg = [&](int u, int cur, float (&a)[4], float (&b)[4][NB]) {
-        const int tap = u / KS, c4 = u % KS;
-        const int ky = tap / 3, kx = tap % 3;
-#pragma unroll
-        for (int gg = 0; gg < 4; ++gg) a[gg] = smem[fa + cur + (tap * CK + c4 * 4) * WS + gg * 16];
-#pragma unroll
-        for (int gg = 0; gg < 4; ++gg) {
-          const int d_ = 1 << gg;
-          const int off = (8 - d_) * (F_PW + 1) + (ky * F_PW + kx) * d_;
-#pragma unroll
-          for (int nb = 0; nb < NB; ++nb) b[gg][nb] = smem[fb + cur + c4 * 4 * F_PS + nb * F_PW + off];
-        }
-      };
-      auto interval_fg = [&](int i, auto par_tag, auto commit_tag, auto issue_tag) {
-        constexpr int PAR = decltype(par_tag)::value;
-        constexpr bool COMMIT = decltype(commit_tag)::value;
-        constexpr int cur = PAR * F_BUF, nxo = (1 - PAR) * F_BUF;
-        if constexpr (COMMIT) load_scales((i + 1) * CK);
-        load_dg(0, cur, ga[0], gb[0]);
-#pragma unroll
-        for (int u = 0; u < NS; ++u) {
-          const int s_ = u & 1;
-          if (u + 1 < NS) load_dg(u + 1, cur, ga[s_ ^ 1], gb[s_ ^ 1]);
-#pragma unroll
-          for (int gg = 0; gg < 4; ++gg)
-#pragma unroll
-            for (int nb = 0; nb < NB; ++nb)
-              acc[gg][nb] = __builtin_amdgcn_mfma_f32_16x16x4f32(ga[s_][gg], gb[s_][gg][nb], acc[gg][nb], 0, 0, 0);
-          staging(u, i, commit_tag, issue_tag, smem + nxo);
-        }
-        __syncthreads();
-      };
-      int iv = 0;
-      for (; iv + 3 < nchunk; iv += 2) {
-        interval_fg(iv, std::integral_constant<int, 0>{}, std::true_type{}, std::true_type{});
-        interval_fg(iv + 1, std::integral_constant<int, 1>{}, std::true_type{}, std::true_type{});
-      }
-      for (; iv < nchunk; ++iv) {
-        const bool c_ = iv + 1 < nchunk, s2 = iv + 2 < nchunk;
-        if (iv & 1) {
-          if (s2) interval_fg(iv, std::integral_constant<int, 1>{}, std::true_type{}, std::true_type{});
-          else if (c_) interval_fg(iv, std::integral_constant<int, 1>{}, std::true_type{}, std::false_type{});
-          else interval_fg(iv, std::integral_constant<int, 1>{}, std::false_type{}, std::false_type{});
-        } else {
-          if (s2) interval_fg(iv, std::integral_constant<int, 0>{}, std::true_type{}, std::true_type{});
-          else if (c_) interval_fg(iv, std::integral_constant<int, 0>{}, std::true_type{}, std::false_type{});
-          else interval_fg(iv, std::integral_constant<int, 0>{}, std::false_type{}, std::false_type{});
-        }
-      }
-    }
-  }
-
+  auto epilogue = [&]() __attribute__((always_inline)) {
+  const ConvK& p = kargs();
+  const int lane_f = fresh_v((int)threadIdx.x) & 63, wave_f = fresh_s(wave);
+  const int lr = lane_f & 15, kq = lane_f >> 4, wm = wave_f / WN, wn = wave_f % WN;
+  const int g = item.g(), co0 = item.co0(), b = item.b(), oy0 = item.oy0, ox0 = item.ox0;
+  const int twl = kind_twl(item.kind()), TW = 1 << twl;
+  const int mlim = (TC && !FG && p.strip_col >= 0 && item.kind() != 2) ? p.H : p.H + 1;
   const int Cout = p.G * p.cout_g;
   const float* osp = p.osp + (int64_t)b * Cout * p.oss;
   const float s1 = p.s1, g1 = p.g1, g2 = p.g2;
@@ -427,6 +434,7 @@
               else
                 yc[yoff[np][py]] = v0;
             }
+          if constexpr (WALK) __builtin_amdgcn_sched_barrier(0);
         }
       }
       return;
@@ -457,6 +465,7 @@
             else
               yc[yoff[np][py]] = v0;
           }
+        if constexpr (WALK) __builtin_amdgcn_sched_barrier(0);
       }
     }
     return;
@@ -506,6 +515,155 @@
         }
       }
     }
+  }
+  };
+
+  if constexpr (WALK) {
+    const int Gs = (int)gridDim.x;
+    const int S = ((p.n_items - 1 - v0) / Gs + 1) * nchunk;
+    PipeItem q0 = item, q1 = item;
+    int qn = 0;
+    int iv = v0, ic = 0;
+    auto open_issue = [&]() __attribute__((always_inline)) {
+      if (ic == nchunk) {
+        ic = 0;
+        iv += Gs;
+        const PipeItem it = make_item(iv);
+        plan_issue(it);
+        if (qn == 0) q0 = it; else q1 = it;
+        ++qn;
+      }
+    };
+    int si = 0;
+    {
+#pragma unroll
+      for (int k = 0; k < NITEM; ++k) issue_item(k, 0);
+      ic = 1;
+      load_scales(i_sbase);
+#pragma unroll
+      for (int k = 0; k < NITEM; ++k) commit_item(k, smem);
+      if (S > 1) {
+        open_issue();
+#pragma unroll
+        for (int k = 0; k < NITEM; ++k) issue_item(k, ic * CK);
+        si = i_sbase + ic * CK * p.wc_cs;
+        ++ic;
+      }
+      __syncthreads();
+    }
+    int mc = 0;
+    for (int s = 0; s < S; ++s) {
+      int ci2 = 0, si2 = si;
+      if (s + 2 < S) {
+        open_issue();
+        ci2 = ic * CK;
+        si2 = i_sbase + ci2 * p.wc_cs;
+        ++ic;
+      } else {
+        xrs = __builtin_amdgcn_make_buffer_rsrc(const_cast<float*>(p.x), 0, 0, 0x00020000);
+        wrs = __builtin_amdgcn_make_buffer_rsrc(const_cast<float*>(p.w), 0, 0, 0x00020000);
+      }
+      interval(s, si, ci2, std::true_type{}, std::true_type{});
+      si = si2;
+      if (++mc == nchunk) {
+        mc = 0;
+        epilogue();
+        clear_acc();
+        item = q0; q0 = q1; --qn;
+        set_mult(item);
+        set_dst();
+      }
+    }
+  } else {
+    {
+#pragma unroll
+      for (int k = 0; k < NITEM; ++k) issue_item(k, 0);
+      load_scales(i_sbase);
+#pragma unroll
+      for (int k = 0; k < NITEM; ++k) commit_item(k, smem);
+      if (nchunk > 1) {
+#pragma unroll
+        for (int k = 0; k < NITEM; ++k) issue_item(k, CK);
+      }
+      __syncthreads();
+    }
+    if constexpr (!FG) {
+      int iv = 0;
+      for (; iv < nchunk - 2; ++iv) interval(iv, i_sbase + (iv + 1) * CK * p.wc_cs, (iv + 2) * CK, std::true_type{}, std::true_type{});
+      if (nchunk >= 2) { interval(iv, i_sbase + (iv + 1) * CK * p.wc_cs, 0, std::true_type{}, std::false_type{}); ++iv; }
+      interval(iv, 0, 0, std::false_type{}, std::false_type{});
+    } else {
+      const int fa = a_lane;
+      const int fb = T * CK * WS + (wn * NP) * F_PW + lr + kq * F_PS;
+      constexpr int NS = T * KS;
+      constexpr int NSI = NS >= 6 ? NS / 3 : 1, NSC = NS - NSI;
+      auto staging = [&](int sidx, int i, auto commit_tag, auto issue_tag, float* nxt) {
+        constexpr bool COMMIT = decltype(commit_tag)::value, ISSUE = decltype(issue_tag)::value;
+        if (COMMIT && sidx < NSC) {
+#pragma unroll
+          for (int k = sidx * NITEM / NSC; k < (sidx + 1) * NITEM / NSC; ++k) commit_item(k, nxt);
+        }
+        if (ISSUE && sidx >= NSC) {
+#pragma unroll
+          for (int k = (sidx - NSC) * NITEM / NSI; k < (sidx - NSC + 1) * NITEM / NSI; ++k) issue_item(k, (i + 2) * CK);
+        }
+        __builtin_amdgcn_sched_barrier(0);
+      };
+      {
+        float ga[2][4], gb[2][4][NB];
+        auto load_dg = [&](int u, int cur, float (&a)[4], float (&b)[4][NB]) {
+          const int tap = u / KS, c4 = u % KS;
+          const int ky = tap / 3, kx = tap % 3;
+#pragma unroll
+          for (int gg = 0; gg < 4; ++gg) a[gg] = smem[fa + cur + (tap * CK + c4 * 4) * WS + gg * 16];
+#pragma unroll
+          for (int gg = 0; gg < 4; ++gg) {
+            const int d_ = 1 << gg;
+            const int off = (8 - d_) * (F_PW + 1) + (ky * F_PW + kx) * d_;
+#pragma unroll
+            for (int nb = 0; nb < NB; ++nb) b[gg][nb] = smem[fb + cur + c4 * 4 * F_PS + nb * F_PW + off];
+          }
+        };
+        auto interval_fg = [&](int i, auto par_tag, auto commit_tag, auto issue_tag) {
+          constexpr int PAR = decltype(par_tag)::value;
+          constexpr bool COMMIT = decltype(commit_tag)::value;
+          constexpr int cur = PAR * F_BUF, nxo = (1 - PAR) * F_BUF;
+          if constexpr (COMMIT) load_scales(i_sbase + (i + 1) * CK * p.wc_cs);
+          load_dg(0, cur, ga[0], gb[0]);
+#pragma unroll
+          for (int u = 0; u < NS; ++u) {
+            const int s_ = u & 1;
+            if (u + 1 < NS) load_dg(u + 1, cur, ga[s_ ^ 1], gb[s_ ^ 1]);
+#pragma unroll
+            for (int gg = 0; gg < 4; ++gg)
+#pragma unroll
+              for (int nb = 0; nb < NB; ++nb)
+                acc[gg][nb] = __builtin_amdgcn_mfma_f32_16x16x4f32(ga[s_][gg], gb[s_][gg][nb], acc[gg][nb], 0, 0, 0);
+            staging(u, i, commit_tag, issue_tag, smem + nxo);
+          }
+          __syncthreads();
+        };
+        int iv = 0;
+        for (; iv + 3 < nchunk; iv += 2) {
+          interval_fg(iv, std::integral_constant<int, 0>{}, std::true_type{}, std::true_type{});
+          interval_fg(iv + 1, std::integral_constant<int, 1>{}, std::true_type{}, std::true_type{});
+        }
+        for (; iv < nchunk; ++iv) {
+          const bool c_ = iv + 1 < nchunk, s2 = iv + 2 < nchunk;
+          if (iv & 1) {
+            if (s2) interval_fg(iv, std::integral_constant<int, 1>{}, std::true_type{}, std::true_type{});
+            else if (c_) interval_fg(iv, std::integral_constant<int, 1>{}, std::true_type{}, std::false_type{});
+            else interval_fg(iv, std::integral_constant<int, 1>{}, std::false_type{}, std::false_type{});
+          } else {
+            if (s2) interval_fg(iv, std::integral_constant<int, 0>{}, std::true_type{}, std::true_type{});
+            else if (c_) interval_fg(iv, std::integral_constant<int, 0>{}, std::true_type{}, std::false_type{});
+            else interval_fg(iv, std::integral_constant<int, 0>{}, std::false_type{}, std::false_type{});
+          }
+        }
+      }
+    }
+
+    epilogue();
   }
 }
 
```
